# choutilin/makani

Hardware: AMD Instinct MI355X
Metric: SFNO fwd+bwd samples/sec, 73ch 721x1440 (higher is better)
Workload: dtype bf16; 1 GPU; sfno_linear_73chq_sc3_layers8_edim384 fwd+bwd+Adam, 73ch 721x1440, per-GPU batch 1; global_batch=1, parallelism=h1, spectral_dtype=f32 (GEMMs as 6 bf16 MFMA products of exact 3-way operand splits), step_launch=eager, micro_batches=1, python_gc=disabled in the timed region, adam=after backward

## Files before the change

include/makani_amd.h:

```cpp
#ifndef MAKANI_AMD_H
#define MAKANI_AMD_H

#include <stdint.h>

#ifdef __cplusplus
extern "C" {
#endif

int mk_version(void);
const char* mk_last_error(void);


int mk_quadrature(int grid, int nlat, double* theta, double* weights);

int mk_legendre_kpad(int nlat);

int mk_legendre_table(int grid, int nlat, int lmax, int mmax, int with_quad_weights, float* out);

int mk_fft_twiddle_len(int nlon);
int mk_fft_twiddles(int nlon, float* out);

int mk_rfft(const void* x, int x_dtype, float* xf, const float* twiddles,
            int bc, int nlat, int nlon, int mmax, float scale0, float scale_m, float scale_h,
            void* stream);

int mk_irfft(const float* xf, void* x, int x_dtype, const float* twiddles,
             int bc, int nlat, int nlon, int mmax, float scale0, float scale_m, float scale_h,
             void* stream);

int mk_legendre_fwd(const float* xf, const float* tab, float* c,
                    int bc, int nlat, int lmax, int mmax_loc, int m_off, int mmax_glob, void* stream);

int mk_legendre_inv(const float* c, const float* tab, float* xf,
                    int bc, int nlat, int lmax, int mmax_loc, int m_off, int mmax_glob, void* stream);

long long mk_legendre_x3_bytes(int nlat, int lmax, int mmax, int inverse);
int mk_legendre_x3_split(const float* tab, void* out, int nlat, int lmax, int mmax, int inverse, void* stream);
int mk_legendre_fwd_x3(const float* xf, const void* tab_x3, float* c,
                       int bc, int nlat, int lmax, int mmax_loc, int m_off, int mmax_glob, void* stream);
int mk_legendre_inv_x3(const float* c, const void* tab_x3, float* xf,
                       int bc, int nlat, int lmax, int mmax_loc, int m_off, int mmax_glob, void* stream);

int mk_rfft_ex(const void* x, int x_dtype, float* xf, const float* twiddles, int bc, int nlat, int nlon,
               int mmax, float scale0, float scale_m, float scale_h, int xf_layout, void* stream);
int mk_irfft_ex(const float* xf, void* x, int x_dtype, const float* twiddles, int bc, int nlat, int nlon,
                int mmax, float scale0, float scale_m, float scale_h, int xf_layout, void* stream);
int mk_legendre_fwd_x3_ex(const float* xf, const void* tab_x3, float* c, int bc, int nlat, int lmax,
                          int mmax_loc, int m_off, int mmax_glob, int xf_layout, void* stream);
int mk_legendre_inv_x3_ex(const float* c, const void* tab_x3, float* xf, int bc, int nlat, int lmax,
                          int mmax_loc, int m_off, int mmax_glob, int xf_layout, void* stream);

int mk_rfft_pm(const void* x, int x_dtype, float* xf, const float* twiddles, int bc, int nlat, int nlon, int mmax,
               float scale0, float scale_m, float scale_h, int chans, int chans_per_peer, void* stream);
int mk_irfft_pm(const float* xf, void* x, int x_dtype, const float* twiddles, int bc, int nlat, int nlon, int mmax,
                float scale0, float scale_m, float scale_h, int chans, int chans_per_peer, void* stream);

int mk_irfft_sums(const float* xf, void* x, int x_dtype, const float* twiddles, int bc, int nlat, int nlon, int mmax,
                  float scale0, float scale_m, float scale_h, int xf_layout, int chans, int chans_per_peer, double* rowsums,
                  void* stream);
int mk_irfft_sums_ws(const float* xf, void* x, int x_dtype, const float* twiddles, int bc, int nlat, int nlon, int mmax,
                     float scale0, float scale_m, float scale_h, int xf_layout, int chans, int chans_per_peer, double* rowsums,
                     double* workspace, void* stream);
int mk_irfft_affine_add(const float* xf, void* x, int x_dtype, const float* twiddles, int bc, int nlat, int nlon,
                        int mmax, float scale0, float scale_m, float scale_h, int xf_layout, const void* z,
                        const float* affine, void* stream);

long long mk_latdft_table_len(int nlat, int lmax);
int mk_latdft_table(int nlat, int lmax, float* out);
int mk_latdft_fwd(const float* xf, const float* table, float* c, int nlat, int lmax, long long ncols, void* stream);
int mk_latdft_inv(const float* c, const float* table, float* xf, int nlat, int lmax, long long ncols, void* stream);

int mk_dhconv_fwd(const float* x, const float* w, float* y, int lloc, int mloc, int batch,
                  int cin, int cout, int l_off, int m_off, void* stream);
int mk_dhconv_dgrad(const float* gy, const float* w, float* gx, int lloc, int mloc, int batch,
                    int cin, int cout, int l_off, int m_off, void* stream);
int mk_dhconv_wgrad(const float* x, const float* gy, float* gw, int lloc, int mloc, int batch,
                    int cin, int cout, int l_off, int m_off, void* stream);

int mk_dhconv_fwd_x3(const float* x, const float* w, float* y, int lloc, int mloc, int batch,
                     int cin, int cout, int l_off, int m_off, void* stream);
int mk_dhconv_dgrad_x3(const float* gy, const float* w, float* gx, int lloc, int mloc, int batch,
                       int cin, int cout, int l_off, int m_off, void* stream);
int mk_dhconv_wgrad_x3(const float* x, const float* gy, float* gw, int lloc, int mloc, int batch,
                       int cin, int cout, int l_off, int m_off, void* stream);

int mk_spec_mix_fwd(const float* x, const float* w, float* y, int lloc, int mloc, int batch,
                    int cin, int cout, int l_off, int m_off, void* stream);
int mk_spec_mix_dgrad(const float* gy, const float* w, float* gx, int lloc, int mloc, int batch,
                      int cin, int cout, int l_off, int m_off, void* stream);
int mk_spec_mix_wgrad(const float* x, const float* gy, float* gw, int lloc, int mloc, int batch,
                      int cin, int cout, int l_off, int m_off, void* stream);

int mk_spec_cmlp_fwd(const float* x, const float* w, const float* bias, float* y, int lloc, int mloc, int batch, int cin,
                     int cout, int l_off, int m_off, int per_degree, int act, void* stream);
int mk_spec_cmlp_dgrad(const float* gy, const float* w, const float* a, float* gx, int lloc, int mloc, int batch, int cin,
                       int cout, int l_off, int m_off, int per_degree, int act, void* stream);
long long mk_spec_cmlp_wgrad_workspace(int lloc, int cin, int cout, int per_degree);
int mk_spec_cmlp_wgrad(const float* x, const float* gy, float* gw, void* workspace, int lloc, int mloc, int batch, int cin,
                       int cout, int l_off, int m_off, int per_degree, void* stream);
long long mk_spec_cmlp_bgrad_workspace(int lloc, int cout);
int mk_spec_cmlp_bgrad(const float* g, float* gb, void* workspace, int lloc, int mloc, int batch, int cout, int l_off,
                       int m_off, void* stream);

int mk_spec_bdmlp_fwd(const float* x, const float* w, float* y, int rows, int nb, int ib, int ob, int act, float lambda,
                      void* stream);
int mk_spec_bdmlp_dgrad(const float* gy, const float* w, const float* a, float* gx, int rows, int nb, int ib, int ob, int act,
                        void* stream);
long long mk_spec_bdmlp_wgrad_workspace(int rows, int nb, int ib, int ob);
int mk_spec_bdmlp_wgrad(const float* x, const float* gy, float* gw, void* workspace, int rows, int nb, int ib, int ob,
                        void* stream);
int mk_spec_bdmlp_mask(const float* gy, const float* s, float* out, long long n, void* stream);

int mk_diag_fwd(const float* x, const float* w, float* y, int batch, int cin, int cout, long long P, void* stream);
int mk_diag_dgrad(const float* gy, const float* w, float* gx, int batch, int cin, int cout, long long P, void* stream);
int mk_diag_wgrad(const float* x, const float* gy, float* gw, int batch, int cin, int cout, long long P, void* stream);

int mk_spec_pack(const float* c_std, float* c_prv, int bc, int lloc, int mloc, void* stream);
int mk_spec_unpack(const float* c_prv, float* c_std, int bc, int lloc, int mloc,
                   int l_off, int m_off, void* stream);

int mk_bias_gelu_fwd(const void* x, const float* bias, void* y, int dtype, int rows, int C, long long P,
                     void* stream);
int mk_bias_gelu_bwd(const void* x, const float* bias, const void* gy, void* gx, float* gbias, int dtype,
                     int rows, int C, long long P, void* stream);
int mk_affine_add(const void* r, const void* z, const float* affine, void* y, int dtype, int rows, long long P,
                  void* stream);
int mk_instnorm_fwd(const void* x, const float* weight, const float* bias, void* y, float* stats,
                    double* workspace, int dtype, int rows, int C, long long P, float eps, int fuse_gelu,
                    void* stream);
int mk_instnorm_bwd(const void* x, const void* gy, const float* stats, const float* weight, const float* bias,
                    void* gx, double* workspace, int dtype, int rows, int C, long long P, int fuse_gelu,
                    void* stream);

int mk_instnorm_fwd_ex(const void* x, const float* weight, const float* bias, void* y, float* stats,
                       double* workspace, int dtype, int rows, int C, long long P, long long count, float eps,
                       int fuse_gelu, int phase, void* stream);
int mk_instnorm_bwd_ex(const void* x, const void* gy, const float* stats, const float* weight, const float* bias,
                       void* gx, double* workspace, int dtype, int rows, int C, long long P, long long count,
                       int fuse_gelu, int phase, void* stream);
int mk_instnorm_bwd_wb(const void* x, const void* gy, const float* stats, const float* weight, const float* bias, void* gx,
                       double* workspace, float* gwb, int dtype, int C, long long P, int fuse_gelu, void* stream);

int mk_wmse_fwd(const void* pred, int dtype, const float* tar, const float* wrow, double* loss, long long rows,
                int H, int W, float scale, void* stream);
int mk_wmse_bwd(const void* pred, int dtype, const float* tar, const float* wrow, const float* gloss, void* gpred,
                long long rows, int H, int W, float scale, void* stream);

int mk_conv1x1_x3(const float* a, long long lda, const float* b, long long ldb, float* c, long long ldc, int M, int K, long long N,
                  int batch, long long sa, long long sb, long long sc, int mode, void* stream);
int mk_conv1x1_x3_bias_act(const float* a, long long lda, const float* b, long long ldb, float* c, long long ldc, int M, int K,
                           long long N, int batch, long long sb, long long sc, const float* bias, int act, void* stream);

int mk_conv1x1_wgrad(const void* gy, const void* x, float* gw, int batch, int cout, int cin, long long P,
                     void* stream);
int mk_conv1x1_wgrad_act(const void* gy, const void* x, float* gw, int batch, int cout, int cin, long long P, int x_act,
                         void* stream);
long long mk_pce_image_bytes(int M, int K);
int mk_pce_pack(const void* w, int w_dtype , int transpose, int M, int K, int ldw, void* img,
                void* stream);
int mk_pce_pack_layout(int M, int K, long long* out3);
int mk_pce_pack_batch(const void* desc_dev, int n, void* arena, long long total_elements, void* stream);
int mk_pce_gemm(const void* x, const void* wimg, void* y, const float* bias, const void* addend, const void* aux_in,
                void* aux_out, int gelu, int batch, int M, int K, long long P, void* stream);
int mk_pce_gemm_ex(const void* x, const void* wimg, void* y, const float* bias, const void* addend, const float* addend_affine,
                   const void* aux_in, void* aux_out, int gelu, double* rowstats, int batch, int M, int K, long long P,
                   void* stream);
long long mk_pce_mlp_image_bytes(int M, int Hd, int K1);
int mk_pce_mlp_pack(const void* a1, int a1_transposed, int lda1, const void* a2, int a2_transposed, int lda2,
                    int w_dtype , int M, int Hd, int K1, void* img, void* stream);
int mk_pce_mlp(const void* x, const void* wimg, void* y, void* mid_out, const void* mid_in, const float* b1, const float* b2,
               double* rowstats_y, double* rowsum_mid, int mode, int batch, int M, int Hd, int K1, long long P, void* stream);
int mk_pce_mlp_debug_stamps(unsigned long long* out512);
int mk_instnorm_coeffs(const double* sums, const float* weight, const float* bias, float* stats, float* affine, int rows,
                       int C, long long count, float eps, void* stream);
int mk_pce_debug_stamps(unsigned long long* out512);

int mk_adam_step(float* p, const float* g, float* m, float* v, long long n, float lr, float beta1, float beta2, float eps,
                 float weight_decay, int step, void* stream);

long long mk_mt_chunks(long long n);
int mk_mt_sumsq(int T, const uint64_t* x, const long long* n, double* partials, double* tsum, int clip_mode, float max_norm,
                float* norm_out, float* coef_out, float* steps, const int* inc_slots, int ninc, void* stream);
int mk_mt_norm_finish(int T, const double* tsum, int clip_mode, float max_norm, float* norm_out, float* coef_out,
                      float* steps, const int* inc_slots, int ninc, void* stream);
int mk_mt_step_inc(float* steps, const int* slots, int nslots, void* stream);
int mk_mt_scale(int T, const uint64_t* x, const long long* n, const float* coef, void* stream);
int mk_mt_adam(int T, const uint64_t* pgmv, const long long* n, const int* step_or_slot, const float* steps, float lr,
               const float* lr_dev, float beta1, float beta2, float eps, float weight_decay, int adamw, const float* coef,
               void* stream);
int mk_mt_lamb(int stage, int T, const uint64_t* pgmv, const long long* n, const int* step_or_slot, const float* steps,
               float lr, const float* lr_dev, float beta1, float beta2, float beta3, float eps, float weight_decay, int adamw,
               int bias_correction, int trust, const float* coef, double* part_p, double* part_u, double* tsum_p,
               double* tsum_u, void* stream);

long long mk_geo_metric_workspace(int B, int C, int H);
int mk_geo_metric_sums(const void* pred, int dtype, const float* tar, const float* clim, const float* wrow, double* workspace,
                       double* sums, int B, int C, int H, int W, void* stream);

long long mk_geo_lp_workspace(int B, int C, int H);
int mk_geo_lp_sums(const void* pred, int dtype, const float* tar, const float* wrow, double* workspace, double* sums, int p,
                   int B, int C, int H, int W, void* stream);
int mk_geo_lp_bwd(const void* pred, int dtype, const float* tar, const float* wrow, const float* g, void* gpred, int p,
                  int B, int C, int H, int W, void* stream);

int mk_input_assemble(const void* x, int x_dtype, const float* u, const float* stat, const float* mean, const float* std,
                      const int* mask_chans, int n_mask, int mask_src, void* out, int out_dtype, int B, int T, int C, int Cu,
                      int Cs, int H, int W, void* stream);
int mk_input_assemble_bwd(const void* gout, int g_dtype, const float* stat, const float* std, const int* mask_chans, int n_mask,
                          int mask_src, void* gx, int x_dtype, int B, int T, int C, int Cu, int Cs, int H, int W, void* stream);

long long mk_history_workspace(int B, int Cn, int H);
int mk_history_sums(const void* x, int x_dtype, const float* u, const float* wt, double* workspace, double* sums, int B, int T,
                    int C, int Cu, int H, int W, void* stream);

int mk_cos_zenith(const float* eph, const float* sin_lat, const float* cos_lat, const float* lon_rad, float* out, long long n,
                  int H, int W, void* stream);

long long mk_chan_layernorm_workspace(int B, int C, long long P);
int mk_chan_layernorm_fwd(const void* x, int x_dtype, const float* weight, const float* bias, void* y, int y_dtype,
                          float* stats, int B, int C, long long P, float eps, int fuse_gelu, void* stream);
int mk_chan_layernorm_bwd(const void* x, int x_dtype, const void* gy, int gy_dtype, const float* stats, const float* weight,
                          const float* bias, void* gx, float* workspace, float* gwb, int B, int C, long long P, int fuse_gelu,
                          void* stream);

long long mk_degree_power_workspace(int L, int M, int BC);
int mk_degree_power(const float* c, double* workspace, double* P, int L, int M, int BC, int l_off, int m_off, void* stream);
int mk_degree_power_bwd(const float* c, const double* gP, float* gc, int L, int M, int BC, int l_off, int m_off, void* stream);

#ifdef __cplusplus
}
#endif
#endif
```

makani_amd/_lib.py:

```python
import ctypes
import os

import torch

from . import build as _build

_LIB = None

_c_int = ctypes.c_int
_c_float = ctypes.c_float
_vp = ctypes.c_void_p

SIGNATURES = {
    "mk_version": (_c_int, []),
    "mk_last_error": (ctypes.c_char_p, []),
    "mk_quadrature": (_c_int, [_c_int, _c_int, _vp, _vp]),
    "mk_legendre_kpad": (_c_int, [_c_int]),
    "mk_legendre_table": (_c_int, [_c_int, _c_int, _c_int, _c_int, _c_int, _vp]),
    "mk_fft_twiddle_len": (_c_int, [_c_int]),
    "mk_fft_twiddles": (_c_int, [_c_int, _vp]),
    "mk_rfft": (_c_int, [_vp, _c_int, _vp, _vp, _c_int, _c_int, _c_int, _c_int, _c_float, _c_float, _c_float, _vp]),
    "mk_irfft": (_c_int, [_vp, _vp, _c_int, _vp, _c_int, _c_int, _c_int, _c_int, _c_float, _c_float, _c_float, _vp]),
    "mk_legendre_fwd": (_c_int, [_vp, _vp, _vp, _c_int, _c_int, _c_int, _c_int, _c_int, _c_int, _vp]),
    "mk_legendre_inv": (_c_int, [_vp, _vp, _vp, _c_int, _c_int, _c_int, _c_int, _c_int, _c_int, _vp]),
    "mk_legendre_x3_bytes": (ctypes.c_longlong, [_c_int, _c_int, _c_int, _c_int]),
    "mk_legendre_x3_split": (_c_int, [_vp, _vp, _c_int, _c_int, _c_int, _c_int, _vp]),
    "mk_legendre_fwd_x3": (_c_int, [_vp, _vp, _vp, _c_int, _c_int, _c_int, _c_int, _c_int, _c_int, _vp]),
    "mk_legendre_inv_x3": (_c_int, [_vp, _vp, _vp, _c_int, _c_int, _c_int, _c_int, _c_int, _c_int, _vp]),
    "mk_rfft_ex": (_c_int, [_vp, _c_int, _vp, _vp, _c_int, _c_int, _c_int, _c_int, _c_float, _c_float, _c_float, _c_int, _vp]),
    "mk_irfft_ex": (_c_int, [_vp, _vp, _c_int, _vp, _c_int, _c_int, _c_int, _c_int, _c_float, _c_float, _c_float, _c_int, _vp]),
    "mk_rfft_pm": (_c_int, [_vp, _c_int, _vp, _vp, _c_int, _c_int, _c_int, _c_int, _c_float, _c_float, _c_float, _c_int, _c_int, _vp]),
    "mk_irfft_pm": (_c_int, [_vp, _vp, _c_int, _vp, _c_int, _c_int, _c_int, _c_int, _c_float, _c_float, _c_float, _c_int, _c_int, _vp]),
    "mk_irfft_sums": (_c_int, [_vp, _vp, _c_int, _vp, _c_int, _c_int, _c_int, _c_int, _c_float, _c_float, _c_float, _c_int, _c_int,
                               _c_int, _vp, _vp]),
    "mk_irfft_sums_ws": (_c_int, [_vp, _vp, _c_int, _vp, _c_int, _c_int, _c_int, _c_int, _c_float, _c_float, _c_float, _c_int, _c_int,
                                  _c_int, _vp, _vp, _vp]),
    "mk_irfft_affine_add": (_c_int, [_vp, _vp, _c_int, _vp, _c_int, _c_int, _c_int, _c_int, _c_float, _c_float, _c_float, _c_int,
                                     _vp, _vp, _vp]),
    "mk_legendre_fwd_x3_ex": (_c_int, [_vp, _vp, _vp, _c_int, _c_int, _c_int, _c_int, _c_int, _c_int, _c_int, _vp]),
    "mk_legendre_inv_x3_ex": (_c_int, [_vp, _vp, _vp, _c_int, _c_int, _c_int, _c_int, _c_int, _c_int, _c_int, _vp]),
    "mk_latdft_table_len": (ctypes.c_longlong, [_c_int, _c_int]),
    "mk_latdft_table": (_c_int, [_c_int, _c_int, _vp]),
    "mk_latdft_fwd": (_c_int, [_vp, _vp, _vp, _c_int, _c_int, ctypes.c_longlong, _vp]),
    "mk_latdft_inv": (_c_int, [_vp, _vp, _vp, _c_int, _c_int, ctypes.c_longlong, _vp]),
    "mk_dhconv_fwd": (_c_int, [_vp, _vp, _vp] + [_c_int] * 7 + [_vp]),
    "mk_dhconv_dgrad": (_c_int, [_vp, _vp, _vp] + [_c_int] * 7 + [_vp]),
    "mk_dhconv_wgrad": (_c_int, [_vp, _vp, _vp] + [_c_int] * 7 + [_vp]),
    "mk_dhconv_fwd_x3": (_c_int, [_vp, _vp, _vp] + [_c_int] * 7 + [_vp]),
    "mk_dhconv_dgrad_x3": (_c_int, [_vp, _vp, _vp] + [_c_int] * 7 + [_vp]),
    "mk_dhconv_wgrad_x3": (_c_int, [_vp, _vp, _vp] + [_c_int] * 7 + [_vp]),
    "mk_spec_mix_fwd": (_c_int, [_vp, _vp, _vp] + [_c_int] * 7 + [_vp]),
    "mk_spec_mix_dgrad": (_c_int, [_vp, _vp, _vp] + [_c_int] * 7 + [_vp]),
    "mk_spec_mix_wgrad": (_c_int, [_vp, _vp, _vp] + [_c_int] * 7 + [_vp]),
    "mk_spec_cmlp_fwd": (_c_int, [_vp, _vp, _vp, _vp] + [_c_int] * 9 + [_vp]),
    "mk_spec_cmlp_dgrad": (_c_int, [_vp, _vp, _vp, _vp] + [_c_int] * 9 + [_vp]),
    "mk_spec_cmlp_wgrad_workspace": (ctypes.c_longlong, [_c_int] * 4),
    "mk_spec_cmlp_wgrad": (_c_int, [_vp, _vp, _vp, _vp] + [_c_int] * 8 + [_vp]),
    "mk_spec_cmlp_bgrad_workspace": (ctypes.c_longlong, [_c_int] * 2),
    "mk_spec_cmlp_bgrad": (_c_int, [_vp, _vp, _vp] + [_c_int] * 6 + [_vp]),
    "mk_spec_bdmlp_fwd": (_c_int, [_vp, _vp, _vp] + [_c_int] * 5 + [_c_float, _vp]),
    "mk_spec_bdmlp_dgrad": (_c_int, [_vp, _vp, _vp, _vp] + [_c_int] * 5 + [_vp]),
    "mk_spec_bdmlp_wgrad_workspace": (ctypes.c_longlong, [_c_int] * 4),
    "mk_spec_bdmlp_wgrad": (_c_int, [_vp, _vp, _vp, _vp] + [_c_int] * 4 + [_vp]),
    "mk_spec_bdmlp_mask": (_c_int, [_vp, _vp, _vp, ctypes.c_longlong, _vp]),
    "mk_affine_add":(_c_int, [_vp, _vp, _vp, _vp, _c_int, _c_int, ctypes.c_longlong, _vp]),
    "mk_diag_fwd": (_c_int, [_vp, _vp, _vp, _c_int, _c_int, _c_int, ctypes.c_longlong, _vp]),
    "mk_diag_dgrad": (_c_int, [_vp, _vp, _vp, _c_int, _c_int, _c_int, ctypes.c_longlong, _vp]),
    "mk_diag_wgrad": (_c_int, [_vp, _vp, _vp, _c_int, _c_int, _c_int, ctypes.c_longlong, _vp]),
    "mk_spec_pack": (_c_int, [_vp, _vp, _c_int, _c_int, _c_int, _vp]),
    "mk_spec_unpack": (_c_int, [_vp, _vp, _c_int, _c_int, _c_int, _c_int, _c_int, _vp]),
    "mk_bias_gelu_fwd": (_c_int, [_vp, _vp, _vp, _c_int, _c_int, _c_int, ctypes.c_longlong, _vp]),
    "mk_bias_gelu_bwd": (_c_int, [_vp, _vp, _vp, _vp, _vp, _c_int, _c_int, _c_int, ctypes.c_longlong, _vp]),
    "mk_instnorm_fwd": (_c_int, [_vp, _vp, _vp, _vp, _vp, _vp, _c_int, _c_int, _c_int, ctypes.c_longlong, _c_float,
                                 _c_int, _vp]),
    "mk_instnorm_fwd_ex": (_c_int, [_vp, _vp, _vp, _vp, _vp, _vp, _c_int, _c_int, _c_int, ctypes.c_longlong,
                                    ctypes.c_longlong, _c_float, _c_int, _c_int, _vp]),
    "mk_instnorm_bwd_ex": (_c_int, [_vp, _vp, _vp, _vp, _vp, _vp, _vp, _c_int, _c_int, _c_int, ctypes.c_longlong,
                                    ctypes.c_longlong, _c_int, _c_int, _vp]),
    "mk_instnorm_bwd_wb": (_c_int, [_vp, _vp, _vp, _vp, _vp, _vp, _vp, _vp, _c_int, _c_int, ctypes.c_longlong, _c_int, _vp]),
    "mk_wmse_fwd": (_c_int, [_vp, _c_int, _vp, _vp, _vp, ctypes.c_longlong, _c_int, _c_int, _c_float, _vp]),
    "mk_wmse_bwd": (_c_int, [_vp, _c_int, _vp, _vp, _vp, _vp, ctypes.c_longlong, _c_int, _c_int, _c_float, _vp]),
    "mk_conv1x1_wgrad": (_c_int, [_vp, _vp, _vp, _c_int, _c_int, _c_int, ctypes.c_longlong, _vp]),
    "mk_conv1x1_x3": (_c_int, [_vp, ctypes.c_longlong, _vp, ctypes.c_longlong, _vp, ctypes.c_longlong, _c_int, _c_int, ctypes.c_longlong,
                               _c_int, ctypes.c_longlong, ctypes.c_longlong, ctypes.c_longlong, _c_int, _vp]),
    "mk_conv1x1_x3_bias_act": (_c_int, [_vp, ctypes.c_longlong, _vp, ctypes.c_longlong, _vp, ctypes.c_longlong, _c_int, _c_int,
                                        ctypes.c_longlong, _c_int, ctypes.c_longlong, ctypes.c_longlong, _vp, _c_int, _vp]),
    "mk_conv1x1_wgrad_act": (_c_int, [_vp, _vp, _vp, _c_int, _c_int, _c_int, ctypes.c_longlong, _c_int, _vp]),
    "mk_pce_mlp_image_bytes": (ctypes.c_longlong, [_c_int, _c_int, _c_int]),
    "mk_pce_mlp_pack": (_c_int, [_vp, _c_int, _c_int, _vp, _c_int, _c_int, _c_int, _c_int, _c_int, _c_int, _vp, _vp]),
    "mk_pce_mlp": (_c_int, [_vp, _vp, _vp, _vp, _vp, _vp, _vp, _vp, _vp, _c_int, _c_int, _c_int, _c_int, _c_int,
                            ctypes.c_longlong, _vp]),
    "mk_pce_mlp_debug_stamps": (_c_int, [_vp]),
    "mk_pce_image_bytes": (ctypes.c_longlong, [_c_int, _c_int]),
    "mk_pce_pack": (_c_int, [_vp, _c_int, _c_int, _c_int, _c_int, _c_int, _vp, _vp]),
    "mk_pce_pack_layout": (_c_int, [_c_int, _c_int, _vp]),
    "mk_pce_pack_batch": (_c_int, [_vp, _c_int, _vp, ctypes.c_longlong, _vp]),
    "mk_pce_gemm": (_c_int, [_vp, _vp, _vp, _vp, _vp, _vp, _vp, _c_int, _c_int, _c_int, _c_int, ctypes.c_longlong, _vp]),
    "mk_pce_gemm_ex": (_c_int, [_vp, _vp, _vp, _vp, _vp, _vp, _vp, _vp, _c_int, _vp, _c_int, _c_int, _c_int, ctypes.c_longlong, _vp]),
    "mk_instnorm_coeffs": (_c_int, [_vp, _vp, _vp, _vp, _vp, _c_int, _c_int, ctypes.c_longlong, ctypes.c_float, _vp]),
    "mk_pce_debug_stamps": (_c_int, [_vp]),
    "mk_adam_step": (_c_int, [_vp, _vp, _vp, _vp, ctypes.c_longlong] + [_c_float] * 5 + [_c_int, _vp]),
    "mk_instnorm_bwd": (_c_int, [_vp, _vp, _vp, _vp, _vp, _vp, _vp, _c_int, _c_int, _c_int, ctypes.c_longlong,
                                 _c_int, _vp]),
    "mk_mt_chunks": (ctypes.c_longlong, [ctypes.c_longlong]),
    "mk_mt_sumsq": (_c_int, [_c_int, _vp, _vp, _vp, _vp, _c_int, _c_float, _vp, _vp, _vp, _vp, _c_int, _vp]),
    "mk_mt_norm_finish": (_c_int, [_c_int, _vp, _c_int, _c_float, _vp, _vp, _vp, _vp, _c_int, _vp]),
    "mk_mt_step_inc": (_c_int, [_vp, _vp, _c_int, _vp]),
    "mk_mt_scale": (_c_int, [_c_int, _vp, _vp, _vp, _vp]),
    "mk_mt_adam": (_c_int, [_c_int, _vp, _vp, _vp, _vp, _c_float, _vp] + [_c_float] * 4 + [_c_int, _vp, _vp]),
    "mk_mt_lamb": (_c_int, [_c_int, _c_int, _vp, _vp, _vp, _vp, _c_float, _vp] + [_c_float] * 5 + [_c_int] * 3
                   + [_vp] * 6),
    "mk_geo_metric_workspace": (ctypes.c_longlong, [_c_int, _c_int, _c_int]),
    "mk_geo_metric_sums": (_c_int, [_vp, _c_int, _vp, _vp, _vp, _vp, _vp, _c_int, _c_int, _c_int, _c_int, _vp]),
    "mk_geo_lp_workspace": (ctypes.c_longlong, [_c_int, _c_int, _c_int]),
    "mk_geo_lp_sums": (_c_int, [_vp, _c_int, _vp, _vp, _vp, _vp] + [_c_int] * 5 + [_vp]),
    "mk_geo_lp_bwd": (_c_int, [_vp, _c_int, _vp, _vp, _vp, _vp] + [_c_int] * 5 + [_vp]),
    "mk_input_assemble": (_c_int, [_vp, _c_int, _vp, _vp, _vp, _vp, _vp, _c_int, _c_int, _vp, _c_int] + [_c_int] * 7 + [_vp]),
    "mk_input_assemble_bwd": (_c_int, [_vp, _c_int, _vp, _vp, _vp, _c_int, _c_int, _vp, _c_int] + [_c_int] * 7 + [_vp]),
    "mk_history_workspace": (ctypes.c_longlong, [_c_int, _c_int, _c_int]),
    "mk_history_sums": (_c_int, [_vp, _c_int, _vp, _vp, _vp, _vp] + [_c_int] * 6 + [_vp]),
    "mk_cos_zenith": (_c_int, [_vp, _vp, _vp, _vp, _vp, ctypes.c_longlong, _c_int, _c_int, _vp]),
    "mk_chan_layernorm_workspace": (ctypes.c_longlong, [_c_int, _c_int, ctypes.c_longlong]),
    "mk_chan_layernorm_fwd": (_c_int, [_vp, _c_int, _vp, _vp, _vp, _c_int, _vp, _c_int, _c_int, ctypes.c_longlong, _c_float,
                                       _c_int, _vp]),
    "mk_chan_layernorm_bwd": (_c_int, [_vp, _c_int, _vp, _c_int, _vp, _vp, _vp, _vp, _vp, _vp, _c_int, _c_int, ctypes.c_longlong,
                                       _c_int, _vp]),
    "mk_degree_power_workspace": (ctypes.c_longlong, [_c_int, _c_int, _c_int]),
    "mk_degree_power": (_c_int, [_vp, _vp, _vp] + [_c_int] * 5 + [_vp]),
    "mk_degree_power_bwd": (_c_int, [_vp, _vp, _vp] + [_c_int] * 5 + [_vp]),
}


def lib_path():
    return _build.LIB


def load():
    global _LIB
    if _LIB is not None:
        return _LIB
    path = _build.LIB
    override = os.environ.get("MK_LIB_OVERRIDE")
    if override:
        path = override
    elif _build.stale():
        if _build.have_hipcc():
            path = _build.build(verbose=False)
        elif not os.path.exists(path):
            raise RuntimeError(f"makani_amd: {path} is missing and hipcc is not available to build it")
        else:
            raise RuntimeError(f"makani_amd: {path} is older than its sources and hipcc is not available to rebuild it")
    try:
        lib = ctypes.CDLL(path)
    except OSError as e:
        raise RuntimeError(f"makani_amd: cannot load the HIP extension {path}: {e}") from e
    for name, (res, args) in SIGNATURES.items():
        fn = getattr(lib, name)
        fn.restype = res
        fn.argtypes = args
    _LIB = lib
    return lib


def check(rc, what=""):
    if rc != 0:
        msg = load().mk_last_error().decode("utf-8", "replace")
        raise RuntimeError(f"makani_amd {what} failed (code {rc}): {msg}")
```

makani_amd/build.py:

```python
import os
import shutil
import subprocess
import sys

HERE = os.path.dirname(os.path.abspath(__file__))
CSRC = os.path.join(HERE, "csrc")
LIB = os.path.join(HERE, "libmakani_amd.so")
STAMP = LIB + ".stamp"
SOURCES = ["host.cpp", "fft.hip", "gemm.hip", "x3_legendre.hip", "x3_spectral.hip", "x3_latdft.hip", "x3_conv.hip", "layout.hip", "diag.hip", "pointwise.hip", "conv_gemm.hip", "pce.hip", "pce_mlp.hip", "adam.hip", "optim.hip", "metrics.hip", "lploss.hip", "preproc.hip", "zenith.hip", "chnorm.hip", "specnorm.hip"]
HEADERS = ["common.h", "x3_engine.h", "fft_split.h", "pce_common.h", "gelu.h", "stream_io.h", "tile_map.h", os.path.join("..", "..", "include", "makani_amd.h")]


def _hipcc():
    for cand in (shutil.which("hipcc"), "/opt/rocm/bin/hipcc"):
        if cand and os.path.exists(cand):
            return cand
    raise RuntimeError("hipcc not found; libmakani_amd.so cannot be built")


def have_hipcc():
    return any(c and os.path.exists(c) for c in (shutil.which("hipcc"), "/opt/rocm/bin/hipcc"))


def _source_digest():
    import hashlib
    h = hashlib.sha256()
    h.update(os.environ.get("MK_EXTRA_HIPCC_FLAGS", "").encode() + b"\0")
    for rel in SOURCES + HEADERS:
        with open(os.path.join(CSRC, rel), "rb") as f:
            h.update(rel.encode() + b"\0" + f.read() + b"\0")
    return h.hexdigest()


def stale():
    if not os.path.exists(LIB) or not os.path.exists(STAMP):
        return True
    with open(STAMP) as f:
        return f.read().strip() != _source_digest()


def build(force=False, verbose=True):
    if not force and not stale():
        return LIB
    hipcc = _hipcc()
    objs = []
    bdir = os.path.join(CSRC, "build")
    os.makedirs(bdir, exist_ok=True)
    procs = []
    for src in SOURCES:
        obj = os.path.join(bdir, src + ".o")
        cmd = [hipcc, "-O3", "-std=c++20", "--offload-arch=gfx950", "-fPIC", "-x", "hip",
               "-c", os.path.join(CSRC, src), "-o", obj] + os.environ.get("MK_EXTRA_HIPCC_FLAGS", "").split()
        if verbose:
            print(" ".join(cmd), flush=True)
        procs.append((src, subprocess.Popen(cmd, stdout=subprocess.PIPE, stderr=subprocess.STDOUT, text=True)))
        objs.append(obj)
    for src, pr in procs:
        out, _ = pr.communicate()
        if pr.returncode != 0:
            raise RuntimeError(f"hipcc failed on {src}:\n{out}")
    cmd = [hipcc, "-shared", "-fPIC", "--offload-arch=gfx950", "-o", LIB] + objs
    if verbose:
        print(" ".join(cmd), flush=True)
    res = subprocess.run(cmd, stdout=subprocess.PIPE, stderr=subprocess.STDOUT, text=True)
    if res.returncode != 0:
        raise RuntimeError(f"link failed:\n{res.stdout}")
    import ctypes
    try:
        ctypes.CDLL(LIB)
    except OSError as e:
        raise RuntimeError(f"{LIB} was linked but does not load: {e}") from e
    with open(STAMP, "w") as f:
        f.write(_source_digest() + "\n")
    return LIB


if __name__ == "__main__":
    print(build(force="--force" in sys.argv))
```

makani_amd/csrc/x3_engine.h:

```cpp
#pragma once
#include "common.h"
#include "tile_map.h"
#include "../../include/makani_amd.h"

#include <cstdint>
#include <cstdlib>

namespace {

typedef float f32x16 __attribute__((ext_vector_type(16)));
typedef __bf16 bf16x8 __attribute__((ext_vector_type(8)));
typedef float x3_f2 __attribute__((ext_vector_type(2)));
typedef float x3_f4 __attribute__((ext_vector_type(4)));

constexpr int XT = 256;
constexpr int XM = 128, XN = 128, XK = 32;
constexpr int XPITCH = 208;
constexpr int XROWB = 192;
constexpr int XIMG = XM * XPITCH + 128;
constexpr int X3_LDS = 2 * XIMG;

__device__ __forceinline__ int plain_off(int r) { return r * XPITCH; }
__device__ __forceinline__ int pair_off(int r) { return ((r >> 1) + ((r & 1) << 6)) * XPITCH + ((r & 1) << 7); }

struct Split3 {
    uint32_t h, m, l;
};
__device__ __forceinline__ Split3 split3(float x) {
    Split3 s;
    s.h = __float_as_uint(x) & 0xFFFF0000u;
    const float r1 = x - __uint_as_float(s.h);
    s.m = __float_as_uint(r1) & 0xFFFF0000u;
    s.l = __float_as_uint(r1 - __uint_as_float(s.m));
    return s;
}
__device__ __forceinline__ uint32_t pack_hi(uint32_t e0, uint32_t e1) { return __builtin_amdgcn_perm(e1, e0, 0x07060302u); }

__device__ __forceinline__ void split_store8(const float (&v)[8], char* dst) {
    Split3 s[8];
#pragma unroll
    for (int i = 0; i < 8; ++i) s[i] = split3(v[i]);
    uint4 h, m, l;
    h.x = pack_hi(s[0].h, s[1].h); h.y = pack_hi(s[2].h, s[3].h); h.z = pack_hi(s[4].h, s[5].h); h.w = pack_hi(s[6].h, s[7].h);
    m.x = pack_hi(s[0].m, s[1].m); m.y = pack_hi(s[2].m, s[3].m); m.z = pack_hi(s[4].m, s[5].m); m.w = pack_hi(s[6].m, s[7].m);
    l.x = pack_hi(s[0].l, s[1].l); l.y = pack_hi(s[2].l, s[3].l); l.z = pack_hi(s[4].l, s[5].l); l.w = pack_hi(s[6].l, s[7].l);
    *reinterpret_cast<uint4*>(dst) = h;
    *reinterpret_cast<uint4*>(dst + 64) = m;
    *reinterpret_cast<uint4*>(dst + 128) = l;
}

constexpr unsigned X3_OOB = 0x80000000u;
__device__ __forceinline__ __amdgpu_buffer_rsrc_t x3_rsrc(const float* base) {
    return __builtin_amdgcn_make_buffer_rsrc(const_cast<float*>(base), 0, 0x7FFFFFFF, 0x00020000);
}
__device__ __forceinline__ float4 x3_load16(__amdgpu_buffer_rsrc_t rs, unsigned off) {
    return __builtin_bit_cast(float4, __builtin_amdgcn_raw_buffer_load_b128(rs, off, 0, 0));
}
__device__ __forceinline__ float2 x3_load8(__amdgpu_buffer_rsrc_t rs, unsigned off) {
    return __builtin_bit_cast(float2, __builtin_amdgcn_raw_buffer_load_b64(rs, off, 0, 0));
}


struct TransStager {
    const float* base;
    long long ldk;
    int k_lo, k_hi, cvalid;
    typedef float2 Regs[8];
    static __device__ __forceinline__ int row_off(int r) { return pair_off(r); }
    __device__ __forceinline__ void gload(int kt, Regs& r, int tid) const {
        const int w = tid >> 6, c = (tid & 63) * 2;
        const int k0 = kt * XK + w * 8;
        const __amdgpu_buffer_rsrc_t rs = x3_rsrc(base + (long long)kt * XK * ldk);
#pragma unroll
        for (int i = 0; i < 8; ++i) {
            const int k = k0 + i;
            const bool ok = k >= k_lo && k < k_hi && c < cvalid;
            r[i] = x3_load8(rs, ok ? (unsigned)(((long long)(w * 8 + i) * ldk + c) * 4) : X3_OOB);
        }
    }
    __device__ __forceinline__ void sstore(const Regs& r, char* img, int tid) const {
        const int w = tid >> 6, t = tid & 63;
        float a[8], b[8];
#pragma unroll
        for (int i = 0; i < 8; ++i) {
            a[i] = r[i].x;
            b[i] = r[i].y;
        }
        split_store8(a, img + t * XPITCH + w * 16);
        split_store8(b, img + (t + 64) * XPITCH + 128 + w * 16);
    }
};

__device__ __forceinline__ int quad_row(int lane) { return ((lane >> 3) & 3) + 8 * (lane >> 5) + 4 * ((lane >> 2) & 1); }

struct RowsBelow {
    static __device__ __forceinline__ bool live(int row, int rows) { return row < rows; }
};
template <class ROWS = RowsBelow>
__device__ __forceinline__ void row8_sstore(const float4 (&r)[4], char* img, int tid, int rows) {
#pragma unroll
    for (int q = 0; q < 2; ++q) {
        const int t = tid + q * XT, row = (t >> 6) * 16 + quad_row(t & 63);
        const float v[8] = {r[2 * q].x, r[2 * q].y, r[2 * q].z, r[2 * q].w, r[2 * q + 1].x, r[2 * q + 1].y, r[2 * q + 1].z, r[2 * q + 1].w};
        if (ROWS::live(row, rows)) split_store8(v, img + row * XPITCH + (t & 3) * 16);
    }
}

struct RowStager {
    const float* base;
    long long ld;
    int rows, kvalid;
    typedef float4 Regs[4];
    static __device__ __forceinline__ int row_off(int r) { return plain_off(r); }
    __device__ __forceinline__ void gload(int kt, Regs& r, int tid) const {
        const __amdgpu_buffer_rsrc_t rs = x3_rsrc(base);
#pragma unroll
        for (int q = 0; q < 2; ++q) {
            const int t = tid + q * XT, row = (t >> 6) * 16 + quad_row(t & 63), k = kt * XK + (t & 3) * 8;
            const unsigned off = (unsigned)(((long long)row * ld + k) * 4);
#pragma unroll
            for (int h = 0; h < 2; ++h)
                r[2 * q + h] = x3_load16(rs, (row < rows && k + 4 * h < kvalid) ? off + 16 * h : X3_OOB);
        }
    }
    __device__ __forceinline__ void sstore(const Regs& r, char* img, int tid) const { row8_sstore(r, img, tid, rows); }
};

__device__ __forceinline__ void x3_mfma_step(const char* As, const char* Bs, const int (&a_off)[2], const int (&b_off)[2],
                                             const bool (&live)[2], f32x16 (&acc)[2][2]) {
    constexpr int PA[6] = {2, 0, 1, 1, 0, 0}, PB[6] = {0, 2, 1, 0, 1, 0};
#pragma unroll
    for (int s = 0; s < 2; ++s) {
        bf16x8 bf[2][3];
#pragma unroll
        for (int b = 0; b < 2; ++b)
#pragma unroll
            for (int p = 0; p < 3; ++p) bf[b][p] = *reinterpret_cast<const bf16x8*>(Bs + b_off[b] + p * 64 + s * 32);
#pragma unroll
        for (int a = 0; a < 2; ++a)
            if (live[a]) {
                bf16x8 af[3];
#pragma unroll
                for (int p = 0; p < 3; ++p) af[p] = *reinterpret_cast<const bf16x8*>(As + a_off[a] + p * 64 + s * 32);
#pragma unroll
                for (int t = 0; t < 6; ++t)
#pragma unroll
                    for (int b = 0; b < 2; ++b)
                        acc[a][b] = __builtin_amdgcn_mfma_f32_32x32x16_bf16(af[PA[t]], bf[b][PB[t]], acc[a][b], 0, 0, 0);
            }
    }
}

template <class AS, class BS, class EPI>
__device__ __forceinline__ void x3_tile(const AS& as, const BS& bs, int kt0, int kt1, int rvalid, int cvalid, EPI epi,
                                        char* lds, int exp = 0) {
    const int tid = threadIdx.x, lane = tid & 63;
    const int wave = __builtin_amdgcn_readfirstlane(tid >> 6);
    const int wr = wave >> 1, wc = wave & 1;
    const int fi = lane & 31, kg = lane >> 5;
    char* As = lds;
    char* Bs = lds + XIMG;

    f32x16 acc[2][2];
#pragma unroll
    for (int a = 0; a < 2; ++a)
#pragma unroll
        for (int b = 0; b < 2; ++b)
#pragma unroll
            for (int r = 0; r < 16; ++r) acc[a][b][r] = 0.f;
    asm volatile("" : "+a"(acc[0][0]), "+a"(acc[0][1]), "+a"(acc[1][0]), "+a"(acc[1][1]));

    bool live[2];
    int a_off[2], b_off[2];
#pragma unroll
    for (int a = 0; a < 2; ++a) {
        a_off[a] = AS::row_off(wr * 64 + a * 32 + fi) + kg * 16;
        b_off[a] = BS::row_off(wc * 64 + 2 * fi + a) + kg * 16;
        if constexpr (EPI::PAIRED_BANDS) live[a] = (wr * 32 < rvalid) && (wc * 64 < cvalid);
        else live[a] = (wr * 64 + a * 32 < rvalid) && (wc * 64 < cvalid);
    }

    typename AS::Regs ra;
    typename BS::Regs rb;
    if (kt0 < kt1) {
        as.gload(kt0, ra, tid);
        bs.gload(kt0, rb, tid);
        as.sstore(ra, As, tid);
        bs.sstore(rb, Bs, tid);
        __syncthreads();
        if (kt0 + 1 < kt1) as.gload(kt0 + 1, ra, tid);
#pragma unroll
        for (int j = 0; j < 1; ++j)
            if (kt0 + 1 + j < kt1) bs.gload(kt0 + 1 + j, rb, tid);
    }
    for (int ktb = kt0; ktb < kt1; ktb += 1) {
#pragma unroll
        for (int j = 0; j < 1; ++j) {
            const int kt = ktb + j;
            if (kt >= kt1) break;
            if (!(exp & 4)) x3_mfma_step(As, Bs, a_off, b_off, live, acc);
            if (kt + 1 < kt1) {
                __syncthreads();
                if (!(exp & 2)) {
                    as.sstore(ra, As, tid);
                    bs.sstore(rb, Bs, tid);
                }
                __syncthreads();
                if (!(exp & 1)) {
                    if (kt + 2 < kt1 && !(exp & 8)) as.gload(kt + 2, ra, tid);
                    if (kt + 1 + 1 < kt1 && !(exp & 16)) bs.gload(kt + 1 + 1, rb, tid);
                }
            }
        }
    }
    epi.store(acc, wr, wc, fi, kg, rvalid, cvalid);
}


struct StoreEpi {
    float* cbase;
    long long ldc;
    static constexpr bool PAIRED_BANDS = false;
    __device__ __forceinline__ void store(const f32x16 (&acc)[2][2], int wr, int wc, int fi, int kg, int rvalid, int cvalid) const {
        const int col = wc * 64 + 2 * fi;
        if (col < cvalid) {
#pragma unroll
            for (int a = 0; a < 2; ++a)
#pragma unroll
                for (int r = 0; r < 16; ++r) {
                    const int row = wr * 64 + a * 32 + (r & 3) + 8 * (r >> 2) + 4 * kg;
                    if (row < rvalid) {
                        x3_f2 v2;
                        v2[0] = acc[a][0][r];
                        v2[1] = acc[a][1][r];
                        __builtin_nontemporal_store(v2, reinterpret_cast<x3_f2*>(cbase + (long long)row * ldc + col));
                    }
                }
        }
    }
};

struct AccumulateEpi {
    float* cbase;
    long long ldc;
    static constexpr bool PAIRED_BANDS = false;
    __device__ __forceinline__ void store(const f32x16 (&acc)[2][2], int wr, int wc, int fi, int kg, int rvalid, int cvalid) const {
        const int col = wc * 64 + 2 * fi;
        if (col < cvalid) {
#pragma unroll
            for (int a = 0; a < 2; ++a)
#pragma unroll
                for (int r = 0; r < 16; ++r) {
                    const int row = wr * 64 + a * 32 + (r & 3) + 8 * (r >> 2) + 4 * kg;
                    if (row < rvalid) {
                        float2* d = reinterpret_cast<float2*>(cbase + (long long)row * ldc + col);
                        const float2 o = *d;
                        *d = make_float2(o.x + acc[a][0][r], o.y + acc[a][1][r]);
                    }
                }
        }
    }
};

struct AtomicEpi {
    float* cbase;
    long long ldc;
    static constexpr bool PAIRED_BANDS = false;
    __device__ __forceinline__ void store(const f32x16 (&acc)[2][2], int wr, int wc, int fi, int kg, int rvalid, int cvalid) const {
        const int col = wc * 64 + 2 * fi;
        if (col < cvalid) {
#pragma unroll
            for (int a = 0; a < 2; ++a)
#pragma unroll
                for (int r = 0; r < 16; ++r) {
                    const int row = wr * 64 + a * 32 + (r & 3) + 8 * (r >> 2) + 4 * kg;
                    if (row < rvalid) {
                        atomicAdd(cbase + (long long)row * ldc + col, acc[a][0][r]);
                        if (col + 1 < cvalid) atomicAdd(cbase + (long long)row * ldc + col + 1, acc[a][1][r]);
                    }
                }
        }
    }
};

using mk::decode_block;
using mk::TileId;
[[maybe_unused]] inline long long grid_blocks(int nbatch, int tiles_m, int tiles_n) {
    return (long long)mk::ceil_div(nbatch, 8) * 8 * tiles_m * tiles_n;
}

[[maybe_unused]] inline int x3_exp() {
    static const int v = [] { const char* e = getenv("MK_X3_EXP"); return e ? atoi(e) : 0; }();
    return v;
}

template <class P>
int x3_launch(const char* who, void (*kernel)(P), long long nblk, void* stream, const P& p) {
    MK_REQUIRE_AS(who, nblk < 2147483647LL, "grid too large");
    hipLaunchKernelGGL(kernel, dim3((unsigned)nblk), dim3(XT), X3_LDS, (hipStream_t)stream, p);
    MK_LAUNCH_CHECK_AS(who);
    return 0;
}

}
```

makani_amd/csrc/x3_legendre.hip:

```cpp
#include "x3_engine.h"

namespace {

struct F32TileStager {
    const char* base;
    typedef float4 Regs[4];
    static constexpr int TILE_BYTES = XM * XK * 4;
    struct AllRows {
        static __device__ __forceinline__ bool live(int, int) { return true; }
    };
    static __device__ __forceinline__ int row_off(int r) { return plain_off(r); }
    __device__ __forceinline__ void gload(int kt, Regs& r, int tid) const {
        const float* p = reinterpret_cast<const float*>(base + (long long)kt * TILE_BYTES);
#pragma unroll
        for (int q = 0; q < 2; ++q) {
            const int t = tid + q * XT, row = (t >> 6) * 16 + quad_row(t & 63);
            const float* pr = p + row * XK + (t & 3) * 8;
            r[2 * q] = *reinterpret_cast<const float4*>(pr);
            r[2 * q + 1] = *reinterpret_cast<const float4*>(pr + 4);
        }
    }
    __device__ __forceinline__ void sstore(const Regs& r, char* img, int tid) const { row8_sstore<AllRows>(r, img, tid, XM); }
};

struct LegX3Params {
    const float* src;
    const char* tab;
    float* dst;
    int K, L, Mloc, m_off, N2;
    int RT;
    int KC;
    int tiles_n;
    int kmajor;
    int exp;
};

__global__ __launch_bounds__(XT, 3) void legendre_fwd_x3_kernel(LegX3Params p) {
    extern __shared__ __attribute__((aligned(16))) char lds_x3[];
    const TileId t = decode_block(p.Mloc, p.RT, p.tiles_n);
    if (!t.valid) return;
    const int m = t.batch, mg = p.m_off + m;
    const int l0 = mg + t.tm * XM;
    if (l0 >= p.L) return;
    const int n0 = t.tn * XN;
    F32TileStager as;
    as.base = p.tab + ((long long)mg * p.RT + t.tm) * p.KC * F32TileStager::TILE_BYTES;
    TransStager bs;
    bs.base = p.src + (p.kmajor ? (long long)m * p.N2 : (long long)m * p.K * p.N2) + n0;
    bs.ldk = p.kmajor ? (long long)p.Mloc * p.N2 : (long long)p.N2;
    bs.k_lo = 0;
    bs.k_hi = p.K;
    bs.cvalid = p.N2 - n0;
    const StoreEpi epi{p.dst + ((long long)l0 * p.Mloc + m) * p.N2 + n0, (long long)p.Mloc * p.N2};
    x3_tile(as, bs, 0, p.KC, p.L - l0, p.N2 - n0, epi, lds_x3, p.exp);
}

__global__ __launch_bounds__(XT, 3) void legendre_inv_x3_kernel(LegX3Params p) {
    extern __shared__ __attribute__((aligned(16))) char lds_x3[];
    const TileId t = decode_block(p.Mloc, p.RT, p.tiles_n);
    if (!t.valid) return;
    const int m = t.batch, mg = p.m_off + m;
    const int k0 = t.tm * XM;
    if (k0 >= p.K) return;
    const int n0 = t.tn * XN;
    F32TileStager as;
    as.base = p.tab + ((long long)mg * p.RT + t.tm) * p.KC * F32TileStager::TILE_BYTES;
    TransStager bs;
    bs.base = p.src + (long long)m * p.N2 + n0;
    bs.ldk = (long long)p.Mloc * p.N2;
    bs.k_lo = mg;
    bs.k_hi = p.L;
    bs.cvalid = p.N2 - n0;
    const int kt0 = mg >> 5;
    const StoreEpi epi{p.kmajor ? p.dst + ((long long)k0 * p.Mloc + m) * p.N2 + n0 : p.dst + ((long long)m * p.K + k0) * p.N2 + n0,
                       p.kmajor ? (long long)p.Mloc * p.N2 : (long long)p.N2};
    x3_tile(as, bs, kt0 < p.KC ? kt0 : p.KC, p.KC, p.K - k0, p.N2 - n0, epi, lds_x3, p.exp);
}

__global__ void legendre_x3_split_kernel(const float* __restrict__ tab, void* __restrict__ out, int K, int KP, int L,
                                         int M, int RT, int KC, int inverse, long long total) {
    const long long idx = (long long)blockIdx.x * blockDim.x + threadIdx.x;
    if (idx >= total) return;
    const int kk = (int)(idx & 31);
    const int r = (int)((idx >> 5) & 127);
    long long blk = idx >> 12;
    const int kc = (int)(blk % KC);
    blk /= KC;
    const int rt = (int)(blk % RT);
    const int m = (int)(blk / RT);
    int l, k;
    if (!inverse) {
        l = m + rt * XM + r;
        k = kc * XK + kk;
    } else {
        k = rt * XM + r;
        l = kc * XK + kk;
    }
    float v = 0.f;
    if (l < L && k < K) v = tab[((long long)m * L + l) * KP + k];
    reinterpret_cast<float*>(out)[idx] = v;
}

void x3_layout(int nlat, int lmax, int inverse, int* RT, int* KC) {
    if (!inverse) {
        *RT = mk::ceil_div(lmax, XM);
        *KC = mk::ceil_div(nlat, XK);
    } else {
        *RT = mk::ceil_div(nlat, XM);
        *KC = mk::ceil_div(lmax, XK);
    }
}

int legendre_x3_launch(const char* who, bool fwd, const float* src, const void* tab, float* dst, int bc, int nlat, int lmax,
                       int mmax_loc, int m_off, int mmax_glob, int xf_layout, void* stream) {
    MK_REQUIRE_AS(who, src && tab && dst, "null pointer");
    MK_REQUIRE_AS(who, bc > 0 && nlat > 0 && lmax > 0 && mmax_loc > 0, "bad sizes");
    MK_REQUIRE_AS(who, m_off >= 0 && m_off + mmax_loc <= mmax_glob, "mode shard out of range");
    MK_REQUIRE_AS(who, xf_layout == 0 || xf_layout == 1, "xf_layout must be 0 ([M][K][BC]) or 1 ([K][M][BC])");
    LegX3Params p;
    p.kmajor = xf_layout;
    p.src = src;
    p.tab = (const char*)tab;
    p.dst = dst;
    p.K = nlat;
    p.L = lmax;
    p.Mloc = mmax_loc;
    p.m_off = m_off;
    p.N2 = 2 * bc;
    x3_layout(nlat, lmax, fwd ? 0 : 1, &p.RT, &p.KC);
    p.tiles_n = mk::ceil_div(p.N2, XN);
    p.exp = x3_exp();
    const long long nblk = grid_blocks(mmax_loc, p.RT, p.tiles_n);
    MK_REQUIRE_AS(who, nblk < 2147483647LL && 33LL * p.Mloc * p.N2 * 4 < (1LL << 31),
               "operand too large: grid over 2^31 blocks, or 33 * mmax_loc * 2 * bc * 4 bytes (one k-step of the data operand) over 2^31");
    return x3_launch(who, fwd ? legendre_fwd_x3_kernel : legendre_inv_x3_kernel, nblk, stream, p);
}

}

extern "C" long long mk_legendre_x3_bytes(int nlat, int lmax, int mmax, int inverse) {
    if (nlat <= 0 || lmax <= 0 || mmax <= 0) return 0;
    int RT, KC;
    x3_layout(nlat, lmax, inverse, &RT, &KC);
    return (long long)mmax * RT * KC * F32TileStager::TILE_BYTES;
}

extern "C" int mk_legendre_x3_split(const float* tab, void* out, int nlat, int lmax, int mmax, int inverse, void* stream) {
    MK_REQUIRE(tab && out, "null pointer");
    MK_REQUIRE(nlat > 0 && lmax > 0 && mmax > 0, "bad sizes");
    int RT, KC;
    x3_layout(nlat, lmax, inverse, &RT, &KC);
    const long long total = (long long)mmax * RT * KC * XM * XK;
    const long long nblk = (total + 255) / 256;
    MK_REQUIRE(nblk < 2147483647LL, "grid too large");
    hipLaunchKernelGGL(legendre_x3_split_kernel, dim3((unsigned)nblk), dim3(256), 0, (hipStream_t)stream, tab,
                       out, nlat, mk_legendre_kpad(nlat), lmax, mmax, RT, KC, inverse, total);
    MK_LAUNCH_CHECK();
    return 0;
}

extern "C" int mk_legendre_fwd_x3_ex(const float* xf, const void* tab_x3, float* c, int bc, int nlat, int lmax,
                                     int mmax_loc, int m_off, int mmax_glob, int xf_layout, void* stream) {
    return legendre_x3_launch(__func__, true, xf, tab_x3, c, bc, nlat, lmax, mmax_loc, m_off, mmax_glob, xf_layout, stream);
}

extern "C" int mk_legendre_fwd_x3(const float* xf, const void* tab_x3, float* c, int bc, int nlat, int lmax, int mmax_loc,
                                  int m_off, int mmax_glob, void* stream) {
    return mk_legendre_fwd_x3_ex(xf, tab_x3, c, bc, nlat, lmax, mmax_loc, m_off, mmax_glob, 0, stream);
}

extern "C" int mk_legendre_inv_x3_ex(const float* c, const void* tab_x3, float* xf, int bc, int nlat, int lmax,
                                     int mmax_loc, int m_off, int mmax_glob, int xf_layout, void* stream) {
    return legendre_x3_launch(__func__, false, c, tab_x3, xf, bc, nlat, lmax, mmax_loc, m_off, mmax_glob, xf_layout, stream);
}

extern "C" int mk_legendre_inv_x3(const float* c, const void* tab_x3, float* xf, int bc, int nlat, int lmax, int mmax_loc,
                                  int m_off, int mmax_glob, void* stream) {
    return mk_legendre_inv_x3_ex(c, tab_x3, xf, bc, nlat, lmax, mmax_loc, m_off, mmax_glob, 0, stream);
}
```

makani_amd/csrc/x3_spectral.hip:

```cpp
#include "x3_engine.h"

namespace {

__device__ __forceinline__ int tri_rows(int Mloc, int B, int l_off, int m_off, int l) {
    int nm = l_off + l - m_off + 1;
    nm = nm < 0 ? 0 : (nm > Mloc ? Mloc : nm);
    return nm * B;
}

struct DegreeWalk {
    long long lpitch;
    int l0, KPL;
    int Mloc, B, l_off, m_off;
    __device__ __forceinline__ const float* step(const float* base, int kt, int w, int& kk0, int& rows) const {
        const int li = kt / KPL, l = l0 + li;
        kk0 = (kt - li * KPL) * (XK / 2) + w * 4;
        rows = tri_rows(Mloc, B, l_off, m_off, l);
        return base + (long long)l * lpitch;
    }
};

template <bool CONJ_B, bool WALK = false>
struct CplxStager {
    const float* base;
    long long ldk;
    int kk_hi = 0, ovalid;
    DegreeWalk walk = {};
    typedef float2 Regs[4];
    static __device__ __forceinline__ int row_off(int r) { return pair_off(r); }
    __device__ __forceinline__ void gload(int kt, Regs& r, int tid) const {
        const int w = __builtin_amdgcn_readfirstlane(tid >> 6), o = tid & 63;
        int kk0, hi;
        const float* b = base;
        if constexpr (WALK) {
            b = walk.step(base, kt, w, kk0, hi);
        } else {
            kk0 = kt * (XK / 2) + w * 4;
            hi = kk_hi;
        }
        const bool ook = o < ovalid;
        const __amdgpu_buffer_rsrc_t rs = x3_rsrc(b);
#pragma unroll
        for (int i = 0; i < 4; ++i)
            r[i] = x3_load8(rs, (ook && kk0 + i < hi) ? (unsigned)((((long long)(kk0 + i)) * ldk + o) * 8) : X3_OOB);
    }
    __device__ __forceinline__ void sstore(const Regs& r, char* img, int tid) const {
        const int w = tid >> 6, t = tid & 63;
        float a[8], b[8];
#pragma unroll
        for (int i = 0; i < 4; ++i) {
            const float re = r[i].x, im = r[i].y;
            a[2 * i] = re;
            a[2 * i + 1] = CONJ_B ? im : -im;
            b[2 * i] = im;
            b[2 * i + 1] = CONJ_B ? -re : re;
        }
        split_store8(a, img + t * XPITCH + w * 16);
        split_store8(b, img + (t + 64) * XPITCH + 128 + w * 16);
    }
};

struct DgradStager {
    const float* base;
    int O, ivalid;
    typedef float4 Regs[2];
    static __device__ __forceinline__ int row_off(int r) { return pair_off(r); }
    __device__ __forceinline__ void gload(int kt, Regs& r, int tid) const {
        const int i = (tid >> 6) * 16 + quad_row(tid & 63), o = kt * (XK / 2) + (tid & 3) * 4;
        const __amdgpu_buffer_rsrc_t rs = x3_rsrc(base);
        const unsigned off = (unsigned)(((long long)i * O + o) * 8);
#pragma unroll
        for (int h = 0; h < 2; ++h) r[h] = x3_load16(rs, (i < ivalid && o + 2 * h < O) ? off + 16 * h : X3_OOB);
    }
    __device__ __forceinline__ void sstore(const Regs& r, char* img, int tid) const {
        const int i = (tid >> 6) * 16 + quad_row(tid & 63), c = tid & 3;
        const float a[8] = {r[0].x, r[0].y, r[0].z, r[0].w, r[1].x, r[1].y, r[1].z, r[1].w};
        const float b[8] = {-r[0].y, r[0].x, -r[0].w, r[0].z, -r[1].y, r[1].x, -r[1].w, r[1].z};
        split_store8(a, img + i * XPITCH + c * 16);
        split_store8(b, img + (i + 64) * XPITCH + 128 + c * 16);
    }
};

template <bool PAIR, bool WALK>
struct ChanKStager {
    const float* base;
    long long C;
    int r_hi = 0, cvalid;
    DegreeWalk walk = {};
    typedef float2 Regs[8];
    static __device__ __forceinline__ int row_off(int r) { return PAIR ? pair_off(r) : plain_off(r); }
    __device__ __forceinline__ void gload(int kt, Regs& r, int tid) const {
        const int w = __builtin_amdgcn_readfirstlane(tid >> 6), t = tid & 63;
        int r0, hi;
        const float* b = base;
        if constexpr (WALK) {
            b = walk.step(base, kt, w, r0, hi);
        } else {
            r0 = kt * (XK / 2) + w * 4;
            hi = r_hi;
        }
        const __amdgpu_buffer_rsrc_t rs = x3_rsrc(b);
#pragma unroll
        for (int e = 0; e < 2; ++e) {
            const int c = t + 64 * e;
            const bool cok = c < cvalid;
#pragma unroll
            for (int j = 0; j < 4; ++j)
                r[4 * e + j] = x3_load8(rs, (cok && r0 + j < hi) ? (unsigned)((((long long)(r0 + j)) * C + c) * 8) : X3_OOB);
        }
    }
    __device__ __forceinline__ void sstore(const Regs& r, char* img, int tid) const {
        const int w = tid >> 6, t = tid & 63;
#pragma unroll
        for (int e = 0; e < 2; ++e) {
            const float v[8] = {r[4 * e].x, r[4 * e].y, r[4 * e + 1].x, r[4 * e + 1].y,
                                r[4 * e + 2].x, r[4 * e + 2].y, r[4 * e + 3].x, r[4 * e + 3].y};
            split_store8(v, img + row_off(t + 64 * e) + w * 16);
        }
    }
};

struct PanelParams {
    const float* a;
    const float* b;
    float* dst;
    const float* bias;
    const float* aux;
    long long ws;
    int Lloc, Mloc, B, I, O, l_off, m_off, tiles_m, tiles_n;
    int act;
    int exp;
    int G, ngroups;
};


struct CplxBiasReluEpi {
    float* cbase;
    long long ldc;
    const float* bias;
    int act;
    static constexpr bool PAIRED_BANDS = false;
    __device__ __forceinline__ CplxBiasReluEpi(const PanelParams& p, long long off, long long ldc_, int n0)
        : cbase(p.dst + off), ldc(ldc_), bias(p.bias ? p.bias + n0 : nullptr), act(p.act) {}
    __device__ __forceinline__ void store(const f32x16 (&acc)[2][2], int wr, int wc, int fi, int kg, int rvalid, int cvalid) const {
        const int col = wc * 64 + 2 * fi;
        if (col < cvalid) {
            const bool relu_re = act >= 1, relu_im = act == 2;
            float b0 = 0.f, b1 = 0.f;
            if (bias) {
                b0 = bias[col];
                b1 = bias[col + 1];
            }
#pragma unroll
            for (int a = 0; a < 2; ++a)
#pragma unroll
                for (int r = 0; r < 16; ++r) {
                    const int row = wr * 64 + a * 32 + (r & 3) + 8 * (r >> 2) + 4 * kg;
                    if (row < rvalid) {
                        x3_f2 v2;
                        v2[0] = acc[a][0][r] + b0;
                        v2[1] = acc[a][1][r] + b1;
                        if (relu_re) v2[0] = v2[0] > 0.f ? v2[0] : 0.f;
                        if (relu_im) v2[1] = v2[1] > 0.f ? v2[1] : 0.f;
                        *reinterpret_cast<x3_f2*>(cbase + (long long)row * ldc + col) = v2;
                    }
                }
        }
    }
};

struct CplxMaskEpi {
    float* cbase;
    long long ldc;
    const float* aux;
    int act;
    static constexpr bool PAIRED_BANDS = false;
    __device__ __forceinline__ CplxMaskEpi(const PanelParams& p, long long off, long long ldc_, int)
        : cbase(p.dst + off), ldc(ldc_), aux(p.aux + off), act(p.act) {}
    __device__ __forceinline__ void store(const f32x16 (&acc)[2][2], int wr, int wc, int fi, int kg, int rvalid, int cvalid) const {
        const int col = wc * 64 + 2 * fi;
        const bool both = act == 2;
        if (col < cvalid) {
#pragma unroll
            for (int a = 0; a < 2; ++a)
#pragma unroll
                for (int r = 0; r < 16; ++r) {
                    const int row = wr * 64 + a * 32 + (r & 3) + 8 * (r >> 2) + 4 * kg;
                    if (row < rvalid) {
                        const long long off = (long long)row * ldc + col;
                        x3_f2 v2;
                        const float2 m = *reinterpret_cast<const float2*>(aux + off);
                        v2[0] = m.x > 0.f ? acc[a][0][r] : 0.f;
                        v2[1] = (!both || m.y > 0.f) ? acc[a][1][r] : 0.f;
                        *reinterpret_cast<x3_f2*>(cbase + off) = v2;
                    }
                }
        }
    }
};

struct PanelStoreEpi : StoreEpi {
    __device__ __forceinline__ PanelStoreEpi(const PanelParams& p, long long off, long long ldc_, int) : StoreEpi{p.dst + off, ldc_} {}
};


template <class EPI, bool ABLATE>
__global__ __launch_bounds__(XT, 3) void dhconv_fwd_x3_kernel(PanelParams p) {
    extern __shared__ __attribute__((aligned(16))) char lds_x3[];
    const TileId t = decode_block(p.Lloc, p.tiles_m, p.tiles_n);
    if (!t.valid) return;
    const int l = p.Lloc - 1 - t.batch;
    const int R = tri_rows(p.Mloc, p.B, p.l_off, p.m_off, l);
    const int r0 = t.tm * XM;
    if (r0 >= R) return;
    const int n0 = t.tn * XN;
    const long long rowbase = (long long)l * p.Mloc * p.B + r0;
    RowStager as;
    as.base = p.a + rowbase * 2 * p.I;
    as.ld = 2 * p.I;
    as.rows = R - r0;
    as.kvalid = 2 * p.I;
    CplxStager<false> bs;
    bs.base = p.b + ((long long)l * p.ws + n0 / 2) * 2;
    bs.ldk = p.O;
    bs.kk_hi = p.I;
    bs.ovalid = p.O - n0 / 2;
    const EPI epi(p, rowbase * 2 * p.O + n0, 2LL * p.O, n0);
    x3_tile(as, bs, 0, (2 * p.I + XK - 1) / XK, R - r0, 2 * p.O - n0, epi, lds_x3, ABLATE ? p.exp : 0);
}

template <class EPI, bool ABLATE>
__global__ __launch_bounds__(XT, 3) void dhconv_dgrad_x3_kernel(PanelParams p) {
    extern __shared__ __attribute__((aligned(16))) char lds_x3[];
    const TileId t = decode_block(p.Lloc, p.tiles_m, p.tiles_n);
    if (!t.valid) return;
    const int l = p.Lloc - 1 - t.batch;
    const int R = tri_rows(p.Mloc, p.B, p.l_off, p.m_off, l);
    const int r0 = t.tm * XM;
    if (r0 >= R) return;
    const int n0 = t.tn * XN;
    const long long rowbase = (long long)l * p.Mloc * p.B + r0;
    RowStager as;
    as.base = p.a + rowbase * 2 * p.O;
    as.ld = 2 * p.O;
    as.rows = R - r0;
    as.kvalid = 2 * p.O;
    DgradStager bs;
    bs.base = p.b + ((long long)l * p.ws + (long long)(n0 / 2) * p.O) * 2;
    bs.O = p.O;
    bs.ivalid = p.I - n0 / 2;
    const EPI epi(p, rowbase * 2 * p.I + n0, 2LL * p.I, n0);
    x3_tile(as, bs, 0, (2 * p.O + XK - 1) / XK, R - r0, 2 * p.I - n0, epi, lds_x3, ABLATE ? p.exp : 0);
}

__global__ __launch_bounds__(XT, 3) void dhconv_wgrad_x3_kernel(PanelParams p) {
    extern __shared__ __attribute__((aligned(16))) char lds_x3[];
    const TileId t = decode_block(p.Lloc, p.tiles_m, p.tiles_n);
    if (!t.valid) return;
    const int l = p.Lloc - 1 - t.batch;
    const int R = tri_rows(p.Mloc, p.B, p.l_off, p.m_off, l);
    const int i0 = t.tm * XM;
    if (i0 >= p.I) return;
    const int n0 = t.tn * XN;
    const long long rowbase = (long long)l * p.Mloc * p.B;
    ChanKStager<false, false> as;
    as.base = p.a + (rowbase * p.I + i0) * 2;
    as.C = p.I;
    as.r_hi = R;
    as.cvalid = p.I - i0;
    CplxStager<true> bs;
    bs.base = p.b + (rowbase * p.O + n0 / 2) * 2;
    bs.ldk = p.O;
    bs.kk_hi = R;
    bs.ovalid = p.O - n0 / 2;
    const StoreEpi epi{p.dst + ((long long)l * p.I + i0) * 2 * p.O + n0, 2LL * p.O};
    x3_tile(as, bs, 0, (2 * R + XK - 1) / XK, p.I - i0, 2 * p.O - n0, epi, lds_x3, p.exp);
}

__global__ __launch_bounds__(XT, 3) void spec_cmlp_wgrad_shared_kernel(PanelParams p) {
    extern __shared__ __attribute__((aligned(16))) char lds_x3[];
    const TileId t = decode_block(p.ngroups, p.tiles_m, p.tiles_n);
    if (!t.valid) return;
    const int g = p.ngroups - 1 - t.batch;
    const int l0 = g * p.G, l1 = l0 + p.G < p.Lloc ? l0 + p.G : p.Lloc;
    const int KPL = (tri_rows(p.Mloc, p.B, p.l_off, p.m_off, l1 - 1) + XK / 2 - 1) / (XK / 2);
    const int i0 = t.tm * XM, n0 = t.tn * XN;
    if (i0 >= p.I) return;
    ChanKStager<false, true> as;
    as.base = p.a + 2 * i0;
    as.C = p.I;
    as.cvalid = p.I - i0;
    as.walk = {2LL * p.Mloc * p.B * p.I, l0, KPL > 0 ? KPL : 1, p.Mloc, p.B, p.l_off, p.m_off};
    CplxStager<true, true> bs;
    bs.base = p.b + n0;
    bs.ldk = p.O;
    bs.ovalid = p.O - n0 / 2;
    bs.walk = as.walk;
    bs.walk.lpitch = 2LL * p.Mloc * p.B * p.O;
    const StoreEpi epi{p.dst + ((long long)g * p.I + i0) * 2 * p.O + n0, 2LL * p.O};
    x3_tile(as, bs, 0, (l1 - l0) * KPL, p.I - i0, 2 * p.O - n0, epi, lds_x3);
}

__global__ void spec_cmlp_group_sum_kernel(const float4* __restrict__ part, float4* __restrict__ dst, long long n4, int ngroups) {
    const long long e = (long long)blockIdx.x * blockDim.x + threadIdx.x;
    if (e >= n4) return;
    float4 s = part[e];
    int g = 1;
    for (; g + 8 <= ngroups; g += 8) {
        float4 v[8];
#pragma unroll
        for (int j = 0; j < 8; ++j) v[j] = part[(long long)(g + j) * n4 + e];
#pragma unroll
        for (int j = 0; j < 8; ++j) {
            s.x += v[j].x;
            s.y += v[j].y;
            s.z += v[j].z;
            s.w += v[j].w;
        }
    }
    for (; g < ngroups; ++g) {
        const float4 v = part[(long long)g * n4 + e];
        s.x += v.x;
        s.y += v.y;
        s.z += v.z;
        s.w += v.w;
    }
    dst[e] = s;
}

__global__ __launch_bounds__(256) void spec_cmlp_bgrad_rows_kernel(const float* __restrict__ g, double* __restrict__ part, int Mloc,
                                                                   int B, int O2, int l_off, int m_off, int chunks) {
    const int l = blockIdx.x / chunks, c = (blockIdx.x - l * chunks) * 256 + threadIdx.x;
    if (c >= O2) return;
    const int R = tri_rows(Mloc, B, l_off, m_off, l);
    const float* p = g + (long long)l * Mloc * B * O2 + c;
    double s[4] = {0.0, 0.0, 0.0, 0.0};
    int r = 0;
    for (; r + 4 <= R; r += 4)
#pragma unroll
        for (int j = 0; j < 4; ++j) s[j] += (double)p[(long long)(r + j) * O2];
    for (int j = 0; r < R; ++r, ++j) s[j] += (double)p[(long long)r * O2];
    part[(long long)l * O2 + c] = (s[0] + s[1]) + (s[2] + s[3]);
}

__global__ void spec_cmlp_bgrad_sum_kernel(const double* __restrict__ part, float* __restrict__ gb, int Lloc, int O2) {
    const int c = blockIdx.x * blockDim.x + threadIdx.x;
    if (c >= O2) return;
    double s = 0.0;
    for (int l = 0; l < Lloc; ++l) s += part[(long long)l * O2 + c];
    gb[c] = (float)s;
}

int cmlp_group_size(int lloc, int cin, int cout) {
    const long long tiles = (long long)mk::ceil_div(cin, XM) * mk::ceil_div(2 * cout, XN);
    const long long G = mk::ceil_div_ll((long long)lloc * tiles, 768LL);
    return (int)(G < 1 ? 1 : G);
}

struct MixParams {
    const float* a;
    const float* w;
    float* dst;
    int Lloc, Mloc, B, Ca, Cd;
    int l_off, m_off, tiles_m, tiles_n;
    int G, ngroups;
};

struct SpecRowStager {
    const float* base;
    long long ld;
    int rows, cvalid;
    typedef float4 Regs[4];
    static __device__ __forceinline__ int row_off(int r) { return pair_off(r); }
    __device__ __forceinline__ void gload(int kt, Regs& r, int tid) const {
        const __amdgpu_buffer_rsrc_t rs = x3_rsrc(base);
        const int row = (tid >> 6) * 16 + quad_row(tid & 63), i = kt * XK + (tid & 3) * 8;
        const unsigned off = (unsigned)(((long long)row * ld + 2 * i) * 4);
#pragma unroll
        for (int h = 0; h < 4; ++h) r[h] = x3_load16(rs, (row < rows && i + 2 * h < cvalid) ? off + 16 * h : X3_OOB);
    }
    __device__ __forceinline__ void sstore(const Regs& r, char* img, int tid) const {
        const int row = (tid >> 6) * 16 + quad_row(tid & 63), c = tid & 3;
        const float re[8] = {r[0].x, r[0].z, r[1].x, r[1].z, r[2].x, r[2].z, r[3].x, r[3].z};
        const float im[8] = {r[0].y, r[0].w, r[1].y, r[1].w, r[2].y, r[2].w, r[3].y, r[3].w};
        if (row < rows) {
            split_store8(re, img + row * XPITCH + c * 16);
            split_store8(im, img + (row + 64) * XPITCH + 128 + c * 16);
        }
    }
};

struct Row2Stager {
    const float* base;
    long long ld;
    int rows, kvalid;
    typedef float2 Regs[8];
    static __device__ __forceinline__ int row_off(int r) { return pair_off(r); }
    __device__ __forceinline__ void gload(int kt, Regs& r, int tid) const {
        const __amdgpu_buffer_rsrc_t rs = x3_rsrc(base);
#pragma unroll
        for (int q = 0; q < 2; ++q) {
            const int t = tid + q * XT, row = (t >> 6) * 16 + quad_row(t & 63), k = kt * XK + (t & 3) * 8;
            const unsigned off = (unsigned)(((long long)row * ld + k) * 4);
#pragma unroll
            for (int h = 0; h < 4; ++h)
                r[4 * q + h] = x3_load8(rs, (row < rows && k + 2 * h < kvalid) ? off + 8 * h : X3_OOB);
        }
    }
    __device__ __forceinline__ void sstore(const Regs& r, char* img, int tid) const {
#pragma unroll
        for (int q = 0; q < 2; ++q) {
            const int t = tid + q * XT, row = (t >> 6) * 16 + quad_row(t & 63);
            const float v[8] = {r[4 * q].x, r[4 * q].y, r[4 * q + 1].x, r[4 * q + 1].y,
                                r[4 * q + 2].x, r[4 * q + 2].y, r[4 * q + 3].x, r[4 * q + 3].y};
            if (row < rows) split_store8(v, img + pair_off(row) + (t & 3) * 16);
        }
    }
};

struct CplxRowsEpi {
    float* cbase;
    long long ldc;
    static constexpr bool PAIRED_BANDS = false;
    __device__ __forceinline__ void store(const f32x16 (&acc)[2][2], int wr, int wc, int fi, int kg, int rvalid, int cvalid) const {
        const int col = wc * 64 + 2 * fi;
        if (col < cvalid) {
#pragma unroll
            for (int a = 0; a < 2; ++a)
#pragma unroll
                for (int r = 0; r < 16; r += 2) {
                    const int row = wr * 64 + a * 32 + (r & 3) + 8 * (r >> 2) + 4 * kg;
                    if (row < rvalid) {
                        x3_f4 v4;
                        v4[0] = acc[a][0][r];
                        v4[1] = acc[a][0][r + 1];
                        v4[2] = acc[a][1][r];
                        v4[3] = acc[a][1][r + 1];
                        __builtin_nontemporal_store(v4, reinterpret_cast<x3_f4*>(cbase + (long long)(row >> 1) * ldc + 2 * col));
                    }
                }
        }
    }
};

template <bool TRANS>
__global__ __launch_bounds__(XT, 3) void spec_mix_x3_kernel(MixParams p) {
    extern __shared__ __attribute__((aligned(16))) char lds_x3[];
    const TileId t = decode_block(p.Lloc, p.tiles_m, p.tiles_n);
    if (!t.valid) return;
    const int l = p.Lloc - 1 - t.batch;
    const int R = tri_rows(p.Mloc, p.B, p.l_off, p.m_off, l);
    const int r0 = t.tm * (XM / 2);
    if (r0 >= R) return;
    const int n0 = t.tn * XN;
    const long long rowbase = (long long)l * p.Mloc * p.B + r0;
    SpecRowStager as;
    as.base = p.a + rowbase * 2 * p.Ca;
    as.ld = 2LL * p.Ca;
    as.rows = R - r0;
    as.cvalid = p.Ca;
    const CplxRowsEpi epi{p.dst + rowbase * 2 * p.Cd + 2 * n0, 2LL * p.Cd};
    const int kts = (p.Ca + XK - 1) / XK;
    if constexpr (TRANS) {
        TransStager bs;
        bs.base = p.w + n0;
        bs.ldk = p.Cd;
        bs.k_lo = 0;
        bs.k_hi = p.Ca;
        bs.cvalid = p.Cd - n0;
        x3_tile(as, bs, 0, kts, 2 * (R - r0), p.Cd - n0, epi, lds_x3);
    } else {
        Row2Stager bs;
        bs.base = p.w + (long long)n0 * p.Ca;
        bs.ld = p.Ca;
        bs.rows = p.Cd - n0;
        bs.kvalid = p.Ca;
        x3_tile(as, bs, 0, kts, 2 * (R - r0), p.Cd - n0, epi, lds_x3);
    }
}

__global__ __launch_bounds__(XT, 3) void spec_mix_wgrad_x3_kernel(MixParams p) {
    extern __shared__ __attribute__((aligned(16))) char lds_x3[];
    const TileId t = decode_block(p.ngroups, p.tiles_m, p.tiles_n);
    if (!t.valid) return;
    const int g = p.ngroups - 1 - t.batch;
    const int l0 = g * p.G, l1 = l0 + p.G < p.Lloc ? l0 + p.G : p.Lloc;
    const int KPL = (tri_rows(p.Mloc, p.B, p.l_off, p.m_off, l1 - 1) + XK / 2 - 1) / (XK / 2);
    if (KPL == 0) return;
    const int o0 = t.tm * XM, i0 = t.tn * XN;
    ChanKStager<false, true> as;
    as.base = p.a + 2 * o0;
    as.C = p.Ca;
    as.cvalid = p.Ca - o0;
    as.walk = {2LL * p.Mloc * p.B * p.Ca, l0, KPL, p.Mloc, p.B, p.l_off, p.m_off};
    ChanKStager<true, true> bs;
    bs.base = p.w + 2 * i0;
    bs.C = p.Cd;
    bs.cvalid = p.Cd - i0;
    bs.walk = as.walk;
    bs.walk.lpitch = 2LL * p.Mloc * p.B * p.Cd;
    const AtomicEpi epi{p.dst + (long long)o0 * p.Cd + i0, p.Cd};
    x3_tile(as, bs, 0, (l1 - l0) * KPL, p.Ca - o0, p.Cd - i0, epi, lds_x3);
}

struct BlockParams {
    const float* a;
    const float* b;
    float* dst;
    const float* aux;
    int rows, nb, ib, ob, tiles_m, tiles_n;
    float lambda;
    int rg, ngroups;
};

constexpr int BD_STORE = 0, BD_RELU = 2, BD_SHRINK = 3, BD_MASK = 4;

template <int MODE>
struct BlockEpi {
    float* cbase;
    long long ldc;
    const float* aux;
    float lambda;
    static constexpr bool PAIRED_BANDS = false;
    static __device__ __forceinline__ float shrink(float v, float l) { return v > l ? v - l : (v < -l ? v + l : 0.f); }
    __device__ __forceinline__ void store(const f32x16 (&acc)[2][2], int wr, int wc, int fi, int kg, int rvalid, int cvalid) const {
        const int col = wc * 64 + 2 * fi;
        if (col < cvalid) {
#pragma unroll
            for (int a = 0; a < 2; ++a)
#pragma unroll
                for (int r = 0; r < 16; ++r) {
                    const int row = wr * 64 + a * 32 + (r & 3) + 8 * (r >> 2) + 4 * kg;
                    if (row < rvalid) {
                        const long long off = (long long)row * ldc + col;
                        x3_f2 v2;
                        v2[0] = acc[a][0][r];
                        v2[1] = acc[a][1][r];
                        if constexpr (MODE == BD_RELU) {
                            v2[0] = v2[0] > 0.f ? v2[0] : 0.f;
                            v2[1] = v2[1] > 0.f ? v2[1] : 0.f;
                        } else if constexpr (MODE == BD_SHRINK) {
                            v2[0] = shrink(v2[0], lambda);
                            v2[1] = shrink(v2[1], lambda);
                        } else if constexpr (MODE == BD_MASK) {
                            const float2 m = *reinterpret_cast<const float2*>(aux + off);
                            v2[0] = m.x > 0.f ? v2[0] : 0.f;
                            v2[1] = m.y > 0.f ? v2[1] : 0.f;
                        }
                        *reinterpret_cast<x3_f2*>(cbase + off) = v2;
                    }
                }
        }
    }
};

template <int MODE>
__global__ __launch_bounds__(XT, 3) void spec_bdmlp_fwd_kernel(BlockParams p) {
    extern __shared__ __attribute__((aligned(16))) char lds_x3[];
    const TileId t = decode_block(p.nb, p.tiles_m, p.tiles_n);
    if (!t.valid) return;
    const int k = t.batch, r0 = t.tm * XM, n0 = t.tn * XN;
    const long long ci = (long long)p.nb * p.ib, co = (long long)p.nb * p.ob;
    RowStager as;
    as.base = p.a + ((long long)r0 * ci + (long long)k * p.ib) * 2;
    as.ld = 2 * ci;
    as.rows = p.rows - r0;
    as.kvalid = 2 * p.ib;
    CplxStager<false> bs;
    bs.base = p.b + ((long long)k * p.ib * p.ob + n0 / 2) * 2;
    bs.ldk = p.ob;
    bs.kk_hi = p.ib;
    bs.ovalid = p.ob - n0 / 2;
    const BlockEpi<MODE> epi{p.dst + ((long long)r0 * co + (long long)k * p.ob) * 2 + n0, 2 * co, nullptr, p.lambda};
    x3_tile(as, bs, 0, (2 * p.ib + XK - 1) / XK, p.rows - r0, 2 * p.ob - n0, epi, lds_x3);
}

template <int MODE>
__global__ __launch_bounds__(XT, 3) void spec_bdmlp_dgrad_kernel(BlockParams p) {
    extern __shared__ __attribute__((aligned(16))) char lds_x3[];
    const TileId t = decode_block(p.nb, p.tiles_m, p.tiles_n);
    if (!t.valid) return;
    const int k = t.batch, r0 = t.tm * XM, n0 = t.tn * XN;
    const long long ci = (long long)p.nb * p.ib, co = (long long)p.nb * p.ob;
    RowStager as;
    as.base = p.a + ((long long)r0 * co + (long long)k * p.ob) * 2;
    as.ld = 2 * co;
    as.rows = p.rows - r0;
    as.kvalid = 2 * p.ob;
    DgradStager bs;
    bs.base = p.b + ((long long)k * p.ib * p.ob + (long long)(n0 / 2) * p.ob) * 2;
    bs.O = p.ob;
    bs.ivalid = p.ib - n0 / 2;
    const long long off = ((long long)r0 * ci + (long long)k * p.ib) * 2 + n0;
    const BlockEpi<MODE> epi{p.dst + off, 2 * ci, MODE == BD_MASK ? p.aux + off : nullptr, 0.f};
    x3_tile(as, bs, 0, (2 * p.ob + XK - 1) / XK, p.rows - r0, 2 * p.ib - n0, epi, lds_x3);
}

__global__ __launch_bounds__(XT, 3) void spec_bdmlp_wgrad_kernel(BlockParams p) {
    extern __shared__ __attribute__((aligned(16))) char lds_x3[];
    const TileId t = decode_block(p.nb * p.ngroups, p.tiles_m, p.tiles_n);
    if (!t.valid) return;
    const int g = t.batch / p.nb, k = t.batch - g * p.nb;
    const int i0 = t.tm * XM, n0 = t.tn * XN;
    const long long ci = (long long)p.nb * p.ib, co = (long long)p.nb * p.ob;
    const long long rbeg = (long long)g * p.rg;
    const int rcnt = p.rows - rbeg < p.rg ? (int)(p.rows - rbeg) : p.rg;
    ChanKStager<false, false> as;
    as.base = p.a + (rbeg * ci + (long long)k * p.ib + i0) * 2;
    as.C = ci;
    as.r_hi = rcnt;
    as.cvalid = p.ib - i0;
    CplxStager<true> bs;
    bs.base = p.b + (rbeg * co + (long long)k * p.ob + n0 / 2) * 2;
    bs.ldk = co;
    bs.kk_hi = rcnt;
    bs.ovalid = p.ob - n0 / 2;
    const StoreEpi epi{p.dst + (((long long)g * p.nb + k) * p.ib + i0) * 2 * p.ob + n0, 2LL * p.ob};
    x3_tile(as, bs, 0, (2 * rcnt + XK - 1) / XK, p.ib - i0, 2 * p.ob - n0, epi, lds_x3);
}

__global__ void spec_bdmlp_mask_kernel(const float4* __restrict__ gy, const float4* __restrict__ s, float4* __restrict__ out,
                                       long long n4) {
    const long long e = (long long)blockIdx.x * blockDim.x + threadIdx.x;
    if (e >= n4) return;
    const float4 g = gy[e], m = s[e];
    out[e] = make_float4(m.x != 0.f ? g.x : 0.f, m.y != 0.f ? g.y : 0.f, m.z != 0.f ? g.z : 0.f, m.w != 0.f ? g.w : 0.f);
}

int bdmlp_group_rows(int rows, int nb, int ib, int ob) {
    const long long tiles = (long long)nb * mk::ceil_div(ib, XM) * mk::ceil_div(2 * ob, XN);
    const long long want = tiles >= 512 ? 1 : 512 / tiles;
    return (int)(mk::ceil_div_ll(mk::ceil_div_ll(rows, want), 16) * 16);
}

}

static int dh_x3_check(const void* a, const void* b, const void* c, int lloc, int mloc, int batch, int cin, int cout,
                       int l_off, int m_off) {
    MK_REQUIRE(a && b && c, "null pointer");
    MK_REQUIRE(lloc > 0 && mloc > 0 && batch > 0 && cin > 0 && cout > 0, "bad sizes");
    MK_REQUIRE(l_off >= 0 && m_off >= 0, "negative shard offset");
    MK_REQUIRE(cin % 2 == 0 && cout % 2 == 0, "the bf16x3 dhconv kernels need even channel counts (use the fp32 kernels)");
    return 0;
}

static PanelParams panel_params(const float* a, const float* b, float* dst, int lloc, int mloc, int batch, int cin, int cout,
                                int l_off, int m_off, int rows_m, int cols, bool per_degree = true) {
    return PanelParams{a, b, dst, nullptr, nullptr, per_degree ? (long long)cin * cout : 0LL, lloc, mloc, batch, cin, cout,
                       l_off, m_off, mk::ceil_div(rows_m, XM), mk::ceil_div(2 * cols, XN), 0, x3_exp(), 1, 0};
}

extern "C" int mk_dhconv_fwd_x3(const float* x, const float* w, float* y, int lloc, int mloc, int batch, int cin,
                                int cout, int l_off, int m_off, void* stream) {
    if (int e = dh_x3_check(x, w, y, lloc, mloc, batch, cin, cout, l_off, m_off)) return e;
    const PanelParams p = panel_params(x, w, y, lloc, mloc, batch, cin, cout, l_off, m_off, mloc * batch, cout);
    return x3_launch(__func__, dhconv_fwd_x3_kernel<PanelStoreEpi, true>, grid_blocks(lloc, p.tiles_m, p.tiles_n), stream, p);
}

extern "C" int mk_dhconv_dgrad_x3(const float* gy, const float* w, float* gx, int lloc, int mloc, int batch, int cin,
                                  int cout, int l_off, int m_off, void* stream) {
    if (int e = dh_x3_check(gy, w, gx, lloc, mloc, batch, cin, cout, l_off, m_off)) return e;
    const PanelParams p = panel_params(gy, w, gx, lloc, mloc, batch, cin, cout, l_off, m_off, mloc * batch, cin);
    return x3_launch(__func__, dhconv_dgrad_x3_kernel<PanelStoreEpi, true>, grid_blocks(lloc, p.tiles_m, p.tiles_n), stream, p);
}

extern "C" int mk_dhconv_wgrad_x3(const float* x, const float* gy, float* gw, int lloc, int mloc, int batch, int cin,
                                  int cout, int l_off, int m_off, void* stream) {
    if (int e = dh_x3_check(x, gy, gw, lloc, mloc, batch, cin, cout, l_off, m_off)) return e;
    const PanelParams p = panel_params(x, gy, gw, lloc, mloc, batch, cin, cout, l_off, m_off, cin, cout);
    return x3_launch(__func__, dhconv_wgrad_x3_kernel, grid_blocks(lloc, p.tiles_m, p.tiles_n), stream, p);
}

static int spec_mix_check(const void* a, const void* b, const void* c, int lloc, int mloc, int batch, int cin, int cout, int l_off,
                          int m_off) {
    MK_REQUIRE(a && b && c, "null pointer");
    MK_REQUIRE(lloc > 0 && mloc > 0 && batch > 0 && cin > 0 && cout > 0, "bad sizes");
    MK_REQUIRE(l_off >= 0 && m_off >= 0, "negative shard offset");
    MK_REQUIRE(cin % 2 == 0 && cout % 2 == 0, "the spectral channel mix needs even channel counts");
    MK_REQUIRE((((uintptr_t)a | (uintptr_t)b | (uintptr_t)c) & 15) == 0, "operands must be 16-byte aligned");
    const long long cmax = cin > cout ? cin : cout;
    MK_REQUIRE((long long)mloc * batch * cmax * 8 < (1LL << 31) && 33LL * cmax * 4 < (1LL << 31),
               "one degree of the spectrum must stay below 2^31 bytes");
    return 0;
}

static int spec_mix_launch(bool trans, const float* a, const float* w, float* dst, int lloc, int mloc, int batch, int ca, int cd,
                           int l_off, int m_off, void* stream) {
    const MixParams p{a, w, dst, lloc, mloc, batch, ca, cd, l_off, m_off, mk::ceil_div(mloc * batch, XM / 2), mk::ceil_div(cd, XN), 1, 0};
    return x3_launch(__func__, trans ? spec_mix_x3_kernel<true> : spec_mix_x3_kernel<false>, grid_blocks(lloc, p.tiles_m, p.tiles_n),
                     stream, p);
}

extern "C" int mk_spec_mix_fwd(const float* x, const float* w, float* y, int lloc, int mloc, int batch, int cin, int cout,
                               int l_off, int m_off, void* stream) {
    if (int e = spec_mix_check(x, w, y, lloc, mloc, batch, cin, cout, l_off, m_off)) return e;
    return spec_mix_launch(false, x, w, y, lloc, mloc, batch, cin, cout, l_off, m_off, stream);
}

extern "C" int mk_spec_mix_dgrad(const float* gy, const float* w, float* gx, int lloc, int mloc, int batch, int cin, int cout,
                                 int l_off, int m_off, void* stream) {
    if (int e = spec_mix_check(gy, w, gx, lloc, mloc, batch, cin, cout, l_off, m_off)) return e;
    return spec_mix_launch(true, gy, w, gx, lloc, mloc, batch, cout, cin, l_off, m_off, stream);
}

extern "C" int mk_spec_mix_wgrad(const float* x, const float* gy, float* gw, int lloc, int mloc, int batch, int cin, int cout,
                                 int l_off, int m_off, void* stream) {
    if (int e = spec_mix_check(x, gy, gw, lloc, mloc, batch, cin, cout, l_off, m_off)) return e;
    MixParams p{gy, x, gw, lloc, mloc, batch, cout, cin, l_off, m_off, mk::ceil_div(cout, XM), mk::ceil_div(cin, XN), 1, 0};
    long long G = (long long)lloc * p.tiles_m * p.tiles_n / 768;
    p.G = (int)(G < 1 ? 1 : (G > 8 ? 8 : G));
    p.ngroups = mk::ceil_div(lloc, p.G);
    return x3_launch(__func__, spec_mix_wgrad_x3_kernel, grid_blocks(p.ngroups, p.tiles_m, p.tiles_n), stream, p);
}

static int spec_cmlp_check(const void* a, const void* b, const void* c, int lloc, int mloc, int batch, int cin, int cout, int l_off,
                           int m_off, int per_degree, int act) {
    if (int e = spec_mix_check(a, b, c, lloc, mloc, batch, cin, cout, l_off, m_off)) return e;
    MK_REQUIRE(per_degree == 0 || per_degree == 1, "per_degree must be 0 (one shared weight panel) or 1");
    MK_REQUIRE((long long)cin * cout * 8 < (1LL << 31), "one weight panel must stay below 2^31 bytes");
    MK_REQUIRE(act >= 0 && act <= 2, "unknown activation (0 none | 1 real | 2 cartesian)");
    return 0;
}

extern "C" int mk_spec_cmlp_fwd(const float* x, const float* w, const float* bias, float* y, int lloc, int mloc, int batch, int cin,
                                int cout, int l_off, int m_off, int per_degree, int act, void* stream) {
    if (int e = spec_cmlp_check(x, w, y, lloc, mloc, batch, cin, cout, l_off, m_off, per_degree, act)) return e;
    MK_REQUIRE(((uintptr_t)bias & 7) == 0, "the bias must be 8-byte aligned");
    PanelParams p = panel_params(x, w, y, lloc, mloc, batch, cin, cout, l_off, m_off, mloc * batch, cout, per_degree);
    p.bias = bias;
    p.act = act;
    return x3_launch(__func__, dhconv_fwd_x3_kernel<CplxBiasReluEpi, false>, grid_blocks(lloc, p.tiles_m, p.tiles_n), stream, p);
}

extern "C" int mk_spec_cmlp_dgrad(const float* gy, const float* w, const float* a, float* gx, int lloc, int mloc, int batch, int cin,
                                  int cout, int l_off, int m_off, int per_degree, int act, void* stream) {
    if (int e = spec_cmlp_check(gy, w, gx, lloc, mloc, batch, cin, cout, l_off, m_off, per_degree, act)) return e;
    MK_REQUIRE(((uintptr_t)a & 15) == 0, "operands must be 16-byte aligned");
    MK_REQUIRE(a == nullptr || act != 0, "a mask operand needs an activation mode (1 real | 2 cartesian)");
    PanelParams p = panel_params(gy, w, gx, lloc, mloc, batch, cin, cout, l_off, m_off, mloc * batch, cin, per_degree);
    p.aux = a;
    p.act = act;
    return x3_launch(__func__, a ? dhconv_dgrad_x3_kernel<CplxMaskEpi, false> : dhconv_dgrad_x3_kernel<PanelStoreEpi, false>,
                     grid_blocks(lloc, p.tiles_m, p.tiles_n), stream, p);
}

extern "C" long long mk_spec_cmlp_wgrad_workspace(int lloc, int cin, int cout, int per_degree) {
    if (per_degree || lloc <= 0 || cin <= 0 || cout <= 0) return 0;
    const int ngroups = mk::ceil_div(lloc, cmlp_group_size(lloc, cin, cout));
    return ngroups > 1 ? (long long)ngroups * cin * cout * 8 : 0;
}

extern "C" int mk_spec_cmlp_wgrad(const float* x, const float* gy, float* gw, void* workspace, int lloc, int mloc, int batch, int cin,
                                  int cout, int l_off, int m_off, int per_degree, void* stream) {
    if (int e = spec_cmlp_check(x, gy, gw, lloc, mloc, batch, cin, cout, l_off, m_off, per_degree, 0)) return e;
    if (per_degree) return mk_dhconv_wgrad_x3(x, gy, gw, lloc, mloc, batch, cin, cout, l_off, m_off, stream);
    PanelParams p = panel_params(x, gy, gw, lloc, mloc, batch, cin, cout, l_off, m_off, cin, cout, false);
    p.G = cmlp_group_size(lloc, cin, cout);
    p.ngroups = mk::ceil_div(lloc, p.G);
    if (p.ngroups > 1) {
        MK_REQUIRE(workspace && ((uintptr_t)workspace & 15) == 0, "the shared weight gradient needs its 16-byte aligned workspace");
        p.dst = static_cast<float*>(workspace);
    }
    if (int e = x3_launch(__func__, spec_cmlp_wgrad_shared_kernel, grid_blocks(p.ngroups, p.tiles_m, p.tiles_n), stream, p)) return e;
    if (p.ngroups > 1) {
        const long long n4 = (long long)cin * cout / 2;
        hipLaunchKernelGGL(spec_cmlp_group_sum_kernel, dim3((unsigned)mk::ceil_div_ll(n4, 256LL)), dim3(256), 0, (hipStream_t)stream,
                           static_cast<const float4*>(workspace), reinterpret_cast<float4*>(gw), n4, p.ngroups);
        MK_LAUNCH_CHECK();
    }
    return 0;
}

extern "C" long long mk_spec_cmlp_bgrad_workspace(int lloc, int cout) {
    return lloc > 0 && cout > 0 ? (long long)lloc * cout * 2 * 8 : 0;
}

extern "C" int mk_spec_cmlp_bgrad(const float* g, float* gb, void* workspace, int lloc, int mloc, int batch, int cout, int l_off,
                                  int m_off, void* stream) {
    if (int e = spec_mix_check(g, gb, workspace, lloc, mloc, batch, cout, cout, l_off, m_off)) return e;
    const int O2 = 2 * cout, chunks = mk::ceil_div(O2, 256);
    MK_REQUIRE((long long)lloc * chunks < 2147483647LL, "grid too large");
    hipLaunchKernelGGL(spec_cmlp_bgrad_rows_kernel, dim3((unsigned)(lloc * chunks)), dim3(256), 0, (hipStream_t)stream, g,
                       static_cast<double*>(workspace), mloc, batch, O2, l_off, m_off, chunks);
    MK_LAUNCH_CHECK();
    hipLaunchKernelGGL(spec_cmlp_bgrad_sum_kernel, dim3((unsigned)mk::ceil_div(O2, 256)), dim3(256), 0, (hipStream_t)stream,
                       static_cast<const double*>(workspace), gb, lloc, O2);
    MK_LAUNCH_CHECK();
    return 0;
}

static int spec_bdmlp_check(const void* a, const void* b, const void* c, int rows, int nb, int ib, int ob) {
    MK_REQUIRE(a && b && c, "null pointer");
    MK_REQUIRE(rows > 0 && nb > 0 && ib > 0 && ob > 0, "bad sizes");
    MK_REQUIRE(ib % 2 == 0 && ob % 2 == 0, "the block MLP needs even block sizes (block offsets must stay 16-byte aligned)");
    MK_REQUIRE((((uintptr_t)a | (uintptr_t)b | (uintptr_t)c) & 15) == 0, "operands must be 16-byte aligned");
    const long long cmax = (long long)nb * (ib > ob ? ib : ob);
    MK_REQUIRE(129LL * cmax * 8 < (1LL << 31) && (long long)ib * ob * 8 < (1LL << 31),
               "one row tile of the spectrum and one weight panel must stay below 2^31 bytes");
    return 0;
}

static BlockParams bdmlp_params(const float* a, const float* b, float* dst, int rows, int nb, int ib, int ob, int rows_m, int cols) {
    return BlockParams{a, b, dst, nullptr, rows, nb, ib, ob, mk::ceil_div(rows_m, XM), mk::ceil_div(2 * cols, XN), 0.f, 0, 1};
}

extern "C" int mk_spec_bdmlp_fwd(const float* x, const float* w, float* y, int rows, int nb, int ib, int ob, int act, float lambda,
                                 void* stream) {
    if (int e = spec_bdmlp_check(x, w, y, rows, nb, ib, ob)) return e;
    MK_REQUIRE(act == 0 || act == 2 || act == 3, "unknown activation (0 none | 2 cartesian ReLU | 3 soft-shrink)");
    MK_REQUIRE(act != 3 || lambda >= 0.f, "the soft-shrink threshold must not be negative");
    BlockParams p = bdmlp_params(x, w, y, rows, nb, ib, ob, rows, ob);
    p.lambda = lambda;
    const long long nblk = grid_blocks(nb, p.tiles_m, p.tiles_n);
    if (act == 2) return x3_launch(__func__, spec_bdmlp_fwd_kernel<BD_RELU>, nblk, stream, p);
    if (act == 3) return x3_launch(__func__, spec_bdmlp_fwd_kernel<BD_SHRINK>, nblk, stream, p);
    return x3_launch(__func__, spec_bdmlp_fwd_kernel<BD_STORE>, nblk, stream, p);
}

extern "C" int mk_spec_bdmlp_dgrad(const float* gy, const float* w, const float* a, float* gx, int rows, int nb, int ib, int ob,
                                   int act, void* stream) {
    if (int e = spec_bdmlp_check(gy, w, gx, rows, nb, ib, ob)) return e;
    MK_REQUIRE(((uintptr_t)a & 15) == 0, "operands must be 16-byte aligned");
    MK_REQUIRE(act == 0 || act == 2, "unknown mask mode (0 none | 2 cartesian ReLU)");
    MK_REQUIRE((a != nullptr) == (act == 2), "the mask operand and the mask mode go together");
    BlockParams p = bdmlp_params(gy, w, gx, rows, nb, ib, ob, rows, ib);
    p.aux = a;
    return x3_launch(__func__, a ? spec_bdmlp_dgrad_kernel<BD_MASK> : spec_bdmlp_dgrad_kernel<BD_STORE>,
                     grid_blocks(nb, p.tiles_m, p.tiles_n), stream, p);
}

extern "C" long long mk_spec_bdmlp_wgrad_workspace(int rows, int nb, int ib, int ob) {
    if (rows <= 0 || nb <= 0 || ib <= 0 || ob <= 0) return 0;
    const int ngroups = mk::ceil_div(rows, bdmlp_group_rows(rows, nb, ib, ob));
    return ngroups > 1 ? (long long)ngroups * nb * ib * ob * 8 : 0;
}

extern "C" int mk_spec_bdmlp_wgrad(const float* x, const float* gy, float* gw, void* workspace, int rows, int nb, int ib, int ob,
                                   void* stream) {
    if (int e = spec_bdmlp_check(x, gy, gw, rows, nb, ib, ob)) return e;
    BlockParams p = bdmlp_params(x, gy, gw, rows, nb, ib, ob, ib, ob);
    p.rg = bdmlp_group_rows(rows, nb, ib, ob);
    p.ngroups = mk::ceil_div(rows, p.rg);
    const long long cmax = (long long)nb * (ib > ob ? ib : ob);
    MK_REQUIRE((p.rg + 16LL) * cmax * 8 < (1LL << 31), "one row group of the spectrum must stay below 2^31 bytes");
    MK_REQUIRE((long long)nb * p.ngroups < 2147483647LL, "too many row groups");
    if (p.ngroups > 1) {
        MK_REQUIRE(workspace && ((uintptr_t)workspace & 15) == 0, "the block weight gradient needs its 16-byte aligned workspace");
        p.dst = static_cast<float*>(workspace);
    }
    if (int e = x3_launch(__func__, spec_bdmlp_wgrad_kernel, grid_blocks(nb * p.ngroups, p.tiles_m, p.tiles_n), stream, p)) return e;
    if (p.ngroups > 1) {
        const long long n4 = (long long)nb * ib * ob / 2;
        hipLaunchKernelGGL(spec_cmlp_group_sum_kernel, dim3((unsigned)mk::ceil_div_ll(n4, 256LL)), dim3(256), 0, (hipStream_t)stream,
                           static_cast<const float4*>(workspace), reinterpret_cast<float4*>(gw), n4, p.ngroups);
        MK_LAUNCH_CHECK();
    }
    return 0;
}

extern "C" int mk_spec_bdmlp_mask(const float* gy, const float* s, float* out, long long n, void* stream) {
    MK_REQUIRE(gy && s && out, "null pointer");
    MK_REQUIRE(n > 0 && n % 4 == 0, "the element count must be a positive multiple of 4 floats");
    MK_REQUIRE((((uintptr_t)gy | (uintptr_t)s | (uintptr_t)out) & 15) == 0, "operands must be 16-byte aligned");
    const long long nblk = mk::ceil_div_ll(n / 4, 256LL);
    MK_REQUIRE(nblk < 2147483647LL, "grid too large");
    hipLaunchKernelGGL(spec_bdmlp_mask_kernel, dim3((unsigned)nblk), dim3(256), 0, (hipStream_t)stream,
                       reinterpret_cast<const float4*>(gy), reinterpret_cast<const float4*>(s), reinterpret_cast<float4*>(out), n / 4);
    MK_LAUNCH_CHECK();
    return 0;
}
```

Measured before the change: 24.08 samples/s.

## Add 256-row tall-tile x3 GEMM path and enable it for dhconv dgrad

Result: no change. 24.08 samples/s, median of 2 (-0.0%).

```diff
diff --git a/include/makani_amd.h b/include/makani_amd.h
--- a/include/makani_amd.h
+++ b/include/makani_amd.h
@@ -49,6 +49,11 @@
                           int mmax_loc, int m_off, int mmax_glob, int xf_layout, void* stream);
 int mk_legendre_inv_x3_ex(const float* c, const void* tab_x3, float* xf, int bc, int nlat, int lmax,
                           int mmax_loc, int m_off, int mmax_glob, int xf_layout, void* stream);
+int mk_x3_tall_route(int family);
+int mk_legendre_fwd_x3_tile(const float* xf, const void* tab_x3, float* c, int bc, int nlat, int lmax,
+                            int mmax_loc, int m_off, int mmax_glob, int xf_layout, int tall, void* stream);
+int mk_legendre_inv_x3_tile(const float* c, const void* tab_x3, float* xf, int bc, int nlat, int lmax,
+                            int mmax_loc, int m_off, int mmax_glob, int xf_layout, int tall, void* stream);
 
 int mk_rfft_pm(const void* x, int x_dtype, float* xf, const float* twiddles, int bc, int nlat, int nlon, int mmax,
                float scale0, float scale_m, float scale_h, int chans, int chans_per_peer, void* stream);
@@ -83,6 +88,10 @@
                        int cin, int cout, int l_off, int m_off, void* stream);
 int mk_dhconv_wgrad_x3(const float* x, const float* gy, float* gw, int lloc, int mloc, int batch,
                        int cin, int cout, int l_off, int m_off, void* stream);
+int mk_dhconv_fwd_x3_tile(const float* x, const float* w, float* y, int lloc, int mloc, int batch,
+                          int cin, int cout, int l_off, int m_off, int tall, void* stream);
+int mk_dhconv_dgrad_x3_tile(const float* gy, const float* w, float* gx, int lloc, int mloc, int batch,
+                            int cin, int cout, int l_off, int m_off, int tall, void* stream);
 
 int mk_spec_mix_fwd(const float* x, const float* w, float* y, int lloc, int mloc, int batch,
                     int cin, int cout, int l_off, int m_off, void* stream);
diff --git a/makani_amd/_lib.py b/makani_amd/_lib.py
--- a/makani_amd/_lib.py
+++ b/makani_amd/_lib.py
@@ -39,6 +39,9 @@
                                      _vp, _vp, _vp]),
     "mk_legendre_fwd_x3_ex": (_c_int, [_vp, _vp, _vp, _c_int, _c_int, _c_int, _c_int, _c_int, _c_int, _c_int, _vp]),
     "mk_legendre_inv_x3_ex": (_c_int, [_vp, _vp, _vp, _c_int, _c_int, _c_int, _c_int, _c_int, _c_int, _c_int, _vp]),
+    "mk_x3_tall_route": (_c_int, [_c_int]),
+    "mk_legendre_fwd_x3_tile": (_c_int, [_vp, _vp, _vp] + [_c_int] * 8 + [_vp]),
+    "mk_legendre_inv_x3_tile": (_c_int, [_vp, _vp, _vp] + [_c_int] * 8 + [_vp]),
     "mk_latdft_table_len": (ctypes.c_longlong, [_c_int, _c_int]),
     "mk_latdft_table": (_c_int, [_c_int, _c_int, _vp]),
     "mk_latdft_fwd": (_c_int, [_vp, _vp, _vp, _c_int, _c_int, ctypes.c_longlong, _vp]),
@@ -49,6 +52,8 @@
     "mk_dhconv_fwd_x3": (_c_int, [_vp, _vp, _vp] + [_c_int] * 7 + [_vp]),
     "mk_dhconv_dgrad_x3": (_c_int, [_vp, _vp, _vp] + [_c_int] * 7 + [_vp]),
     "mk_dhconv_wgrad_x3": (_c_int, [_vp, _vp, _vp] + [_c_int] * 7 + [_vp]),
+    "mk_dhconv_fwd_x3_tile": (_c_int, [_vp, _vp, _vp] + [_c_int] * 8 + [_vp]),
+    "mk_dhconv_dgrad_x3_tile": (_c_int, [_vp, _vp, _vp] + [_c_int] * 8 + [_vp]),
     "mk_spec_mix_fwd": (_c_int, [_vp, _vp, _vp] + [_c_int] * 7 + [_vp]),
     "mk_spec_mix_dgrad": (_c_int, [_vp, _vp, _vp] + [_c_int] * 7 + [_vp]),
     "mk_spec_mix_wgrad": (_c_int, [_vp, _vp, _vp] + [_c_int] * 7 + [_vp]),
diff --git a/makani_amd/build.py b/makani_amd/build.py
--- a/makani_amd/build.py
+++ b/makani_amd/build.py
@@ -7,8 +7,8 @@
 CSRC = os.path.join(HERE, "csrc")
 LIB = os.path.join(HERE, "libmakani_amd.so")
 STAMP = LIB + ".stamp"
-SOURCES = ["host.cpp", "fft.hip", "gemm.hip", "x3_legendre.hip", "x3_spectral.hip", "x3_latdft.hip", "x3_conv.hip", "layout.hip", "diag.hip", "pointwise.hip", "conv_gemm.hip", "pce.hip", "pce_mlp.hip", "adam.hip", "optim.hip", "metrics.hip", "lploss.hip", "preproc.hip", "zenith.hip", "chnorm.hip", "specnorm.hip"]
-HEADERS = ["common.h", "x3_engine.h", "fft_split.h", "pce_common.h", "gelu.h", "stream_io.h", "tile_map.h", os.path.join("..", "..", "include", "makani_amd.h")]
+SOURCES = ["host.cpp", "fft.hip", "gemm.hip", "x3_legendre.hip", "x3_legendre_tall.hip", "x3_spectral.hip", "x3_spectral_tall.hip", "x3_latdft.hip", "x3_conv.hip", "layout.hip", "diag.hip", "pointwise.hip", "conv_gemm.hip", "pce.hip", "pce_mlp.hip", "adam.hip", "optim.hip", "metrics.hip", "lploss.hip", "preproc.hip", "zenith.hip", "chnorm.hip", "specnorm.hip"]
+HEADERS = ["common.h", "x3_engine.h", "x3_legendre.h", "x3_spectral.h", "fft_split.h", "pce_common.h", "gelu.h", "stream_io.h", "tile_map.h", os.path.join("..", "..", "include", "makani_amd.h")]
 
 
 def _hipcc():
diff --git a/makani_amd/csrc/x3_engine.h b/makani_amd/csrc/x3_engine.h
--- a/makani_amd/csrc/x3_engine.h
+++ b/makani_amd/csrc/x3_engine.h
@@ -3,6 +3,7 @@
 #include "tile_map.h"
 #include "../../include/makani_amd.h"
 
+#include <atomic>
 #include <cstdint>
 #include <cstdlib>
 
@@ -216,6 +217,95 @@
     epi.store(acc, wr, wc, fi, kg, rvalid, cvalid);
 }
 
+constexpr int X3_LDS_TALL = 3 * XIMG;
+
+template <class AS, class BS, class EPI>
+__device__ __forceinline__ void x3_tile_tall(const AS& as0, const AS& as1, const BS& bs, int kt0, int kt1, int rvalid, int cvalid,
+                                             const EPI& epi0, const EPI& epi1, char* lds) {
+    static_assert(!EPI::PAIRED_BANDS, "the tall tile takes epilogues whose 32-row bands are independent");
+    const int tid = threadIdx.x, lane = tid & 63;
+    const int wave = __builtin_amdgcn_readfirstlane(tid >> 6);
+    const int wr = wave >> 1, wc = wave & 1;
+    const int fi = lane & 31, kg = lane >> 5;
+    char* A0 = lds;
+    char* A1 = lds + XIMG;
+    char* Bs = lds + 2 * XIMG;
+    const bool two = rvalid > XM;
+
+    f32x16 acc[2][2][2];
+#pragma unroll
+    for (int i = 0; i < 2; ++i)
+#pragma unroll
+        for (int a = 0; a < 2; ++a)
+#pragma unroll
+            for (int b = 0; b < 2; ++b)
+#pragma unroll
+                for (int r = 0; r < 16; ++r) acc[i][a][b][r] = 0.f;
+    asm volatile("" : "+a"(acc[0][0][0]), "+a"(acc[0][0][1]), "+a"(acc[0][1][0]), "+a"(acc[0][1][1]),
+                      "+a"(acc[1][0][0]), "+a"(acc[1][0][1]), "+a"(acc[1][1][0]), "+a"(acc[1][1][1]));
+
+    bool live0[2], live1[2];
+    int a_off[2], b_off[2];
+#pragma unroll
+    for (int a = 0; a < 2; ++a) {
+        a_off[a] = AS::row_off(wr * 64 + a * 32 + fi) + kg * 16;
+        b_off[a] = BS::row_off(wc * 64 + 2 * fi + a) + kg * 16;
+        live0[a] = (wr * 64 + a * 32 < rvalid) && (wc * 64 < cvalid);
+        live1[a] = (XM + wr * 64 + a * 32 < rvalid) && (wc * 64 < cvalid);
+    }
+
+    typename AS::Regs ra0, ra1;
+    typename BS::Regs rb;
+    if (kt0 < kt1) {
+        as0.gload(kt0, ra0, tid);
+        if (two) as1.gload(kt0, ra1, tid);
+        bs.gload(kt0, rb, tid);
+        as0.sstore(ra0, A0, tid);
+        if (two) as1.sstore(ra1, A1, tid);
+        bs.sstore(rb, Bs, tid);
+        __syncthreads();
+        if (kt0 + 1 < kt1) {
+            as0.gload(kt0 + 1, ra0, tid);
+            if (two) as1.gload(kt0 + 1, ra1, tid);
+            bs.gload(kt0 + 1, rb, tid);
+        }
+    }
+    for (int kt = kt0; kt < kt1; ++kt) {
+        x3_mfma_step(A0, Bs, a_off, b_off, live0, acc[0]);
+        if (two) x3_mfma_step(A1, Bs, a_off, b_off, live1, acc[1]);
+        if (kt + 1 < kt1) {
+            int ts = tid, tg = tid;
+            __syncthreads();
+            asm volatile("" : "+v"(ts));
+            as0.sstore(ra0, A0, ts);
+            if (two) as1.sstore(ra1, A1, ts);
+            bs.sstore(rb, Bs, ts);
+            __syncthreads();
+            if (kt + 2 < kt1) {
+                asm volatile("" : "+v"(tg));
+                as0.gload(kt + 2, ra0, tg);
+                if (two) as1.gload(kt + 2, ra1, tg);
+                bs.gload(kt + 2, rb, tg);
+            }
+        }
+    }
+    int te = tid;
+    asm volatile("" : "+v"(te));
+    const int fie = te & 31, kge = (te & 63) >> 5;
+#pragma unroll
+    for (int i = 0; i < 2; ++i) {
+        if (i == 1 && !two) break;
+        f32x16 c[2][2];
+#pragma unroll
+        for (int a = 0; a < 2; ++a)
+#pragma unroll
+            for (int b = 0; b < 2; ++b) c[a][b] = acc[i][a][b];
+        asm volatile("" : "+v"(c[0][0]), "+v"(c[0][1]), "+v"(c[1][0]), "+v"(c[1][1]) : : "memory");
+        if (i == 0) epi0.store(c, wr, wc, fie, kge, rvalid, cvalid);
+        else epi1.store(c, wr, wc, fie, kge, rvalid - XM, cvalid);
+    }
+}
+
 
 struct StoreEpi {
     float* cbase;
@@ -302,4 +392,27 @@
     return 0;
 }
 
-}
+template <auto Kernel, class P>
+int x3_launch_tall(const char* who, long long nblk, void* stream, const P& p) {
+    MK_REQUIRE_AS(who, nblk < 2147483647LL, "grid too large");
+    static std::atomic<unsigned long long> raised{0};
+    int dev = 0;
+    MK_REQUIRE_AS(who, hipGetDevice(&dev) == hipSuccess && dev >= 0 && dev < 64, "no current device");
+    if (!(raised.load(std::memory_order_acquire) & (1ULL << dev))) {
+        MK_REQUIRE_AS(who, hipFuncSetAttribute(reinterpret_cast<const void*>(Kernel), hipFuncAttributeMaxDynamicSharedMemorySize,
+                                               X3_LDS_TALL) == hipSuccess, "cannot raise the dynamic LDS limit of a tall-tile kernel");
+        raised.fetch_or(1ULL << dev, std::memory_order_release);
+    }
+    hipLaunchKernelGGL(Kernel, dim3((unsigned)nblk), dim3(XT), X3_LDS_TALL, (hipStream_t)stream, p);
+    MK_LAUNCH_CHECK_AS(who);
+    return 0;
+}
+
+constexpr bool X3_TALL_LEGENDRE_FWD = false, X3_TALL_LEGENDRE_INV = false, X3_TALL_DHCONV_FWD = false, X3_TALL_DHCONV_DGRAD = true;
+constexpr int X3_TALL_DHCONV_MODE = 1;
+[[maybe_unused]] inline bool x3_tall_auto(bool family_default) {
+    static const int v = [] { const char* e = getenv("MK_X3_TALL"); return e && *e ? (atoi(e) != 0 ? 1 : 0) : -1; }();
+    return v < 0 ? family_default : v != 0;
+}
+
+}
diff --git a/makani_amd/csrc/x3_legendre.h b/makani_amd/csrc/x3_legendre.h
--- /dev/null
+++ b/makani_amd/csrc/x3_legendre.h
@@ -0,0 +1,73 @@
+#pragma once
+#include "x3_engine.h"
+
+namespace {
+
+struct F32TileStager {
+    const char* base;
+    typedef float4 Regs[4];
+    static constexpr int TILE_BYTES = XM * XK * 4;
+    struct AllRows {
+        static __device__ __forceinline__ bool live(int, int) { return true; }
+    };
+    static __device__ __forceinline__ int row_off(int r) { return plain_off(r); }
+    __device__ __forceinline__ void gload(int kt, Regs& r, int tid) const {
+        const float* p = reinterpret_cast<const float*>(base + (long long)kt * TILE_BYTES);
+#pragma unroll
+        for (int q = 0; q < 2; ++q) {
+            const int t = tid + q * XT, row = (t >> 6) * 16 + quad_row(t & 63);
+            const float* pr = p + row * XK + (t & 3) * 8;
+            r[2 * q] = *reinterpret_cast<const float4*>(pr);
+            r[2 * q + 1] = *reinterpret_cast<const float4*>(pr + 4);
+        }
+    }
+    __device__ __forceinline__ void sstore(const Regs& r, char* img, int tid) const { row8_sstore<AllRows>(r, img, tid, XM); }
+};
+
+struct LegX3Params {
+    const float* src;
+    const char* tab;
+    float* dst;
+    int K, L, Mloc, m_off, N2;
+    int RT;
+    int KC;
+    int tiles_n;
+    int kmajor;
+    int exp;
+};
+
+[[maybe_unused]] inline void x3_layout(int nlat, int lmax, int inverse, int* RT, int* KC) {
+    if (!inverse) {
+        *RT = mk::ceil_div(lmax, XM);
+        *KC = mk::ceil_div(nlat, XK);
+    } else {
+        *RT = mk::ceil_div(nlat, XM);
+        *KC = mk::ceil_div(lmax, XK);
+    }
+}
+
+
+[[maybe_unused]] inline LegX3Params legendre_x3_params(bool fwd, const float* src, const void* tab, float* dst, int bc, int nlat,
+                                                       int lmax, int mmax_loc, int m_off, int xf_layout) {
+    LegX3Params p;
+    p.kmajor = xf_layout;
+    p.src = src;
+    p.tab = (const char*)tab;
+    p.dst = dst;
+    p.K = nlat;
+    p.L = lmax;
+    p.Mloc = mmax_loc;
+    p.m_off = m_off;
+    p.N2 = 2 * bc;
+    x3_layout(nlat, lmax, fwd ? 0 : 1, &p.RT, &p.KC);
+    p.tiles_n = mk::ceil_div(p.N2, XN);
+    p.exp = x3_exp();
+    return p;
+}
+
+}
+
+namespace mk {
+int legendre_x3_tall_launch(const char* who, bool fwd, const float* src, const void* tab, float* dst, int bc, int nlat, int lmax,
+                            int mmax_loc, int m_off, int xf_layout, void* stream);
+}
diff --git a/makani_amd/csrc/x3_legendre.hip b/makani_amd/csrc/x3_legendre.hip
--- a/makani_amd/csrc/x3_legendre.hip
+++ b/makani_amd/csrc/x3_legendre.hip
@@ -1,39 +1,6 @@
-#include "x3_engine.h"
+#include "x3_legendre.h"
 
 namespace {
-
-struct F32TileStager {
-    const char* base;
-    typedef float4 Regs[4];
-    static constexpr int TILE_BYTES = XM * XK * 4;
-    struct AllRows {
-        static __device__ __forceinline__ bool live(int, int) { return true; }
-    };
-    static __device__ __forceinline__ int row_off(int r) { return plain_off(r); }
-    __device__ __forceinline__ void gload(int kt, Regs& r, int tid) const {
-        const float* p = reinterpret_cast<const float*>(base + (long long)kt * TILE_BYTES);
-#pragma unroll
-        for (int q = 0; q < 2; ++q) {
-            const int t = tid + q * XT, row = (t >> 6) * 16 + quad_row(t & 63);
-            const float* pr = p + row * XK + (t & 3) * 8;
-            r[2 * q] = *reinterpret_cast<const float4*>(pr);
-            r[2 * q + 1] = *reinterpret_cast<const float4*>(pr + 4);
-        }
-    }
-    __device__ __forceinline__ void sstore(const Regs& r, char* img, int tid) const { row8_sstore<AllRows>(r, img, tid, XM); }
-};
-
-struct LegX3Params {
-    const float* src;
-    const char* tab;
-    float* dst;
-    int K, L, Mloc, m_off, N2;
-    int RT;
-    int KC;
-    int tiles_n;
-    int kmajor;
-    int exp;
-};
 
 __global__ __launch_bounds__(XT, 3) void legendre_fwd_x3_kernel(LegX3Params p) {
     extern __shared__ __attribute__((aligned(16))) char lds_x3[];
@@ -101,38 +68,19 @@
     reinterpret_cast<float*>(out)[idx] = v;
 }
 
-void x3_layout(int nlat, int lmax, int inverse, int* RT, int* KC) {
-    if (!inverse) {
-        *RT = mk::ceil_div(lmax, XM);
-        *KC = mk::ceil_div(nlat, XK);
-    } else {
-        *RT = mk::ceil_div(nlat, XM);
-        *KC = mk::ceil_div(lmax, XK);
-    }
-}
-
 int legendre_x3_launch(const char* who, bool fwd, const float* src, const void* tab, float* dst, int bc, int nlat, int lmax,
-                       int mmax_loc, int m_off, int mmax_glob, int xf_layout, void* stream) {
+                       int mmax_loc, int m_off, int mmax_glob, int xf_layout, int tall, void* stream) {
     MK_REQUIRE_AS(who, src && tab && dst, "null pointer");
     MK_REQUIRE_AS(who, bc > 0 && nlat > 0 && lmax > 0 && mmax_loc > 0, "bad sizes");
     MK_REQUIRE_AS(who, m_off >= 0 && m_off + mmax_loc <= mmax_glob, "mode shard out of range");
     MK_REQUIRE_AS(who, xf_layout == 0 || xf_layout == 1, "xf_layout must be 0 ([M][K][BC]) or 1 ([K][M][BC])");
-    LegX3Params p;
-    p.kmajor = xf_layout;
-    p.src = src;
-    p.tab = (const char*)tab;
-    p.dst = dst;
-    p.K = nlat;
-    p.L = lmax;
-    p.Mloc = mmax_loc;
-    p.m_off = m_off;
-    p.N2 = 2 * bc;
-    x3_layout(nlat, lmax, fwd ? 0 : 1, &p.RT, &p.KC);
-    p.tiles_n = mk::ceil_div(p.N2, XN);
-    p.exp = x3_exp();
+    MK_REQUIRE_AS(who, tall >= -1 && tall <= 1, "tall must be -1 (auto), 0 (128-row tile) or 1 (256-row tile)");
+    const LegX3Params p = legendre_x3_params(fwd, src, tab, dst, bc, nlat, lmax, mmax_loc, m_off, xf_layout);
+    if (tall < 0) tall = p.RT > 1 && x3_tall_auto(fwd ? X3_TALL_LEGENDRE_FWD : X3_TALL_LEGENDRE_INV);
     const long long nblk = grid_blocks(mmax_loc, p.RT, p.tiles_n);
     MK_REQUIRE_AS(who, nblk < 2147483647LL && 33LL * p.Mloc * p.N2 * 4 < (1LL << 31),
                "operand too large: grid over 2^31 blocks, or 33 * mmax_loc * 2 * bc * 4 bytes (one k-step of the data operand) over 2^31");
+    if (tall) return mk::legendre_x3_tall_launch(who, fwd, src, tab, dst, bc, nlat, lmax, mmax_loc, m_off, xf_layout, stream);
     return x3_launch(who, fwd ? legendre_fwd_x3_kernel : legendre_inv_x3_kernel, nblk, stream, p);
 }
 
@@ -159,9 +107,24 @@
     return 0;
 }
 
+extern "C" int mk_x3_tall_route(int family) {
+    switch (family) {
+        case 0: return x3_tall_auto(X3_TALL_LEGENDRE_FWD) ? 1 : 0;
+        case 1: return x3_tall_auto(X3_TALL_LEGENDRE_INV) ? 1 : 0;
+        case 2: return x3_tall_auto(X3_TALL_DHCONV_FWD) ? X3_TALL_DHCONV_MODE : 0;
+        case 3: return x3_tall_auto(X3_TALL_DHCONV_DGRAD) ? X3_TALL_DHCONV_MODE : 0;
+        default: return -1;
+    }
+}
+
+extern "C" int mk_legendre_fwd_x3_tile(const float* xf, const void* tab_x3, float* c, int bc, int nlat, int lmax,
+                                       int mmax_loc, int m_off, int mmax_glob, int xf_layout, int tall, void* stream) {
+    return legendre_x3_launch(__func__, true, xf, tab_x3, c, bc, nlat, lmax, mmax_loc, m_off, mmax_glob, xf_layout, tall, stream);
+}
+
 extern "C" int mk_legendre_fwd_x3_ex(const float* xf, const void* tab_x3, float* c, int bc, int nlat, int lmax,
                                      int mmax_loc, int m_off, int mmax_glob, int xf_layout, void* stream) {
-    return legendre_x3_launch(__func__, true, xf, tab_x3, c, bc, nlat, lmax, mmax_loc, m_off, mmax_glob, xf_layout, stream);
+    return legendre_x3_launch(__func__, true, xf, tab_x3, c, bc, nlat, lmax, mmax_loc, m_off, mmax_glob, xf_layout, -1, stream);
 }
 
 extern "C" int mk_legendre_fwd_x3(const float* xf, const void* tab_x3, float* c, int bc, int nlat, int lmax, int mmax_loc,
@@ -169,9 +132,14 @@
     return mk_legendre_fwd_x3_ex(xf, tab_x3, c, bc, nlat, lmax, mmax_loc, m_off, mmax_glob, 0, stream);
 }
 
+extern "C" int mk_legendre_inv_x3_tile(const float* c, const void* tab_x3, float* xf, int bc, int nlat, int lmax,
+                                       int mmax_loc, int m_off, int mmax_glob, int xf_layout, int tall, void* stream) {
+    return legendre_x3_launch(__func__, false, c, tab_x3, xf, bc, nlat, lmax, mmax_loc, m_off, mmax_glob, xf_layout, tall, stream);
+}
+
 extern "C" int mk_legendre_inv_x3_ex(const float* c, const void* tab_x3, float* xf, int bc, int nlat, int lmax,
                                      int mmax_loc, int m_off, int mmax_glob, int xf_layout, void* stream) {
-    return legendre_x3_launch(__func__, false, c, tab_x3, xf, bc, nlat, lmax, mmax_loc, m_off, mmax_glob, xf_layout, stream);
+    return legendre_x3_launch(__func__, false, c, tab_x3, xf, bc, nlat, lmax, mmax_loc, m_off, mmax_glob, xf_layout, -1, stream);
 }
 
 extern "C" int mk_legendre_inv_x3(const float* c, const void* tab_x3, float* xf, int bc, int nlat, int lmax, int mmax_loc,
diff --git a/makani_amd/csrc/x3_legendre_tall.hip b/makani_amd/csrc/x3_legendre_tall.hip
--- /dev/null
+++ b/makani_amd/csrc/x3_legendre_tall.hip
@@ -0,0 +1,60 @@
+#include "x3_legendre.h"
+
+namespace {
+
+__global__ __launch_bounds__(XT, 2) void legendre_fwd_x3_tall_kernel(LegX3Params p) {
+    extern __shared__ __attribute__((aligned(16))) char lds_x3[];
+    const TileId t = decode_block(p.Mloc, (p.RT + 1) / 2, p.tiles_n);
+    if (!t.valid) return;
+    const int m = t.batch, mg = p.m_off + m;
+    const int l0 = mg + t.tm * 2 * XM;
+    if (l0 >= p.L) return;
+    const int n0 = t.tn * XN;
+    F32TileStager as0, as1;
+    as0.base = p.tab + ((long long)mg * p.RT + 2 * t.tm) * p.KC * F32TileStager::TILE_BYTES;
+    as1.base = as0.base + (long long)p.KC * F32TileStager::TILE_BYTES;
+    TransStager bs;
+    bs.base = p.src + (p.kmajor ? (long long)m * p.N2 : (long long)m * p.K * p.N2) + n0;
+    bs.ldk = p.kmajor ? (long long)p.Mloc * p.N2 : (long long)p.N2;
+    bs.k_lo = 0;
+    bs.k_hi = p.K;
+    bs.cvalid = p.N2 - n0;
+    const long long ldc = (long long)p.Mloc * p.N2;
+    const StoreEpi epi0{p.dst + ((long long)l0 * p.Mloc + m) * p.N2 + n0, ldc};
+    const StoreEpi epi1{epi0.cbase + XM * ldc, ldc};
+    x3_tile_tall(as0, as1, bs, 0, p.KC, p.L - l0, p.N2 - n0, epi0, epi1, lds_x3);
+}
+
+__global__ __launch_bounds__(XT, 2) void legendre_inv_x3_tall_kernel(LegX3Params p) {
+    extern __shared__ __attribute__((aligned(16))) char lds_x3[];
+    const TileId t = decode_block(p.Mloc, (p.RT + 1) / 2, p.tiles_n);
+    if (!t.valid) return;
+    const int m = t.batch, mg = p.m_off + m;
+    const int k0 = t.tm * 2 * XM;
+    if (k0 >= p.K) return;
+    const int n0 = t.tn * XN;
+    F32TileStager as0, as1;
+    as0.base = p.tab + ((long long)mg * p.RT + 2 * t.tm) * p.KC * F32TileStager::TILE_BYTES;
+    as1.base = as0.base + (long long)p.KC * F32TileStager::TILE_BYTES;
+    TransStager bs;
+    bs.base = p.src + (long long)m * p.N2 + n0;
+    bs.ldk = (long long)p.Mloc * p.N2;
+    bs.k_lo = mg;
+    bs.k_hi = p.L;
+    bs.cvalid = p.N2 - n0;
+    const int kt0 = mg >> 5;
+    const long long ldc = p.kmajor ? (long long)p.Mloc * p.N2 : (long long)p.N2;
+    const StoreEpi epi0{p.kmajor ? p.dst + ((long long)k0 * p.Mloc + m) * p.N2 + n0 : p.dst + ((long long)m * p.K + k0) * p.N2 + n0, ldc};
+    const StoreEpi epi1{epi0.cbase + XM * ldc, ldc};
+    x3_tile_tall(as0, as1, bs, kt0 < p.KC ? kt0 : p.KC, p.KC, p.K - k0, p.N2 - n0, epi0, epi1, lds_x3);
+}
+
+}
+
+int mk::legendre_x3_tall_launch(const char* who, bool fwd, const float* src, const void* tab, float* dst, int bc, int nlat,
+                                int lmax, int mmax_loc, int m_off, int xf_layout, void* stream) {
+    const LegX3Params p = legendre_x3_params(fwd, src, tab, dst, bc, nlat, lmax, mmax_loc, m_off, xf_layout);
+    const long long nblk = grid_blocks(mmax_loc, (p.RT + 1) / 2, p.tiles_n);
+    return fwd ? x3_launch_tall<legendre_fwd_x3_tall_kernel>(who, nblk, stream, p)
+               : x3_launch_tall<legendre_inv_x3_tall_kernel>(who, nblk, stream, p);
+}
diff --git a/makani_amd/csrc/x3_spectral.h b/makani_amd/csrc/x3_spectral.h
--- /dev/null
+++ b/makani_amd/csrc/x3_spectral.h
@@ -0,0 +1,113 @@
+#pragma once
+#include "x3_engine.h"
+
+namespace {
+
+__device__ __forceinline__ int tri_rows(int Mloc, int B, int l_off, int m_off, int l) {
+    int nm = l_off + l - m_off + 1;
+    nm = nm < 0 ? 0 : (nm > Mloc ? Mloc : nm);
+    return nm * B;
+}
+
+struct DegreeWalk {
+    long long lpitch;
+    int l0, KPL;
+    int Mloc, B, l_off, m_off;
+    __device__ __forceinline__ const float* step(const float* base, int kt, int w, int& kk0, int& rows) const {
+        const int li = kt / KPL, l = l0 + li;
+        kk0 = (kt - li * KPL) * (XK / 2) + w * 4;
+        rows = tri_rows(Mloc, B, l_off, m_off, l);
+        return base + (long long)l * lpitch;
+    }
+};
+
+template <bool CONJ_B, bool WALK = false>
+struct CplxStager {
+    const float* base;
+    long long ldk;
+    int kk_hi = 0, ovalid;
+    DegreeWalk walk = {};
+    typedef float2 Regs[4];
+    static __device__ __forceinline__ int row_off(int r) { return pair_off(r); }
+    __device__ __forceinline__ void gload(int kt, Regs& r, int tid) const {
+        const int w = __builtin_amdgcn_readfirstlane(tid >> 6), o = tid & 63;
+        int kk0, hi;
+        const float* b = base;
+        if constexpr (WALK) {
+            b = walk.step(base, kt, w, kk0, hi);
+        } else {
+            kk0 = kt * (XK / 2) + w * 4;
+            hi = kk_hi;
+        }
+        const bool ook = o < ovalid;
+        const __amdgpu_buffer_rsrc_t rs = x3_rsrc(b);
+#pragma unroll
+        for (int i = 0; i < 4; ++i)
+            r[i] = x3_load8(rs, (ook && kk0 + i < hi) ? (unsigned)((((long long)(kk0 + i)) * ldk + o) * 8) : X3_OOB);
+    }
+    __device__ __forceinline__ void sstore(const Regs& r, char* img, int tid) const {
+        const int w = tid >> 6, t = tid & 63;
+        float a[8], b[8];
+#pragma unroll
+        for (int i = 0; i < 4; ++i) {
+            const float re = r[i].x, im = r[i].y;
+            a[2 * i] = re;
+            a[2 * i + 1] = CONJ_B ? im : -im;
+            b[2 * i] = im;
+            b[2 * i + 1] = CONJ_B ? -re : re;
+        }
+        split_store8(a, img + t * XPITCH + w * 16);
+        split_store8(b, img + (t + 64) * XPITCH + 128 + w * 16);
+    }
+};
+
+struct DgradStager {
+    const float* base;
+    int O, ivalid;
+    typedef float4 Regs[2];
+    static __device__ __forceinline__ int row_off(int r) { return pair_off(r); }
+    __device__ __forceinline__ void gload(int kt, Regs& r, int tid) const {
+        const int i = (tid >> 6) * 16 + quad_row(tid & 63), o = kt * (XK / 2) + (tid & 3) * 4;
+        const __amdgpu_buffer_rsrc_t rs = x3_rsrc(base);
+        const unsigned off = (unsigned)(((long long)i * O + o) * 8);
+#pragma unroll
+        for (int h = 0; h < 2; ++h) r[h] = x3_load16(rs, (i < ivalid && o + 2 * h < O) ? off + 16 * h : X3_OOB);
+    }
+    __device__ __forceinline__ void sstore(const Regs& r, char* img, int tid) const {
+        const int i = (tid >> 6) * 16 + quad_row(tid & 63), c = tid & 3;
+        const float a[8] = {r[0].x, r[0].y, r[0].z, r[0].w, r[1].x, r[1].y, r[1].z, r[1].w};
+        const float b[8] = {-r[0].y, r[0].x, -r[0].w, r[0].z, -r[1].y, r[1].x, -r[1].w, r[1].z};
+        split_store8(a, img + i * XPITCH + c * 16);
+        split_store8(b, img + (i + 64) * XPITCH + 128 + c * 16);
+    }
+};
+
+struct PanelParams {
+    const float* a;
+    const float* b;
+    float* dst;
+    const float* bias;
+    const float* aux;
+    long long ws;
+    int Lloc, Mloc, B, I, O, l_off, m_off, tiles_m, tiles_n;
+    int act;
+    int exp;
+    int G, ngroups;
+};
+
+struct PanelStoreEpi : StoreEpi {
+    __device__ __forceinline__ PanelStoreEpi(const PanelParams& p, long long off, long long ldc_, int) : StoreEpi{p.dst + off, ldc_} {}
+};
+
+[[maybe_unused]] inline PanelParams panel_params(const float* a, const float* b, float* dst, int lloc, int mloc, int batch, int cin, int cout,
+                                int l_off, int m_off, int rows_m, int cols, bool per_degree = true) {
+    return PanelParams{a, b, dst, nullptr, nullptr, per_degree ? (long long)cin * cout : 0LL, lloc, mloc, batch, cin, cout,
+                       l_off, m_off, mk::ceil_div(rows_m, XM), mk::ceil_div(2 * cols, XN), 0, x3_exp(), 1, 0};
+}
+
+}
+
+namespace mk {
+int dhconv_x3_tall_launch(const char* who, bool fwd, const float* a, const float* w, float* dst, int lloc, int mloc, int batch,
+                          int cin, int cout, int l_off, int m_off, int nheavy, void* stream);
+}
diff --git a/makani_amd/csrc/x3_spectral.hip b/makani_amd/csrc/x3_spectral.hip
--- a/makani_amd/csrc/x3_spectral.hip
+++ b/makani_amd/csrc/x3_spectral.hip
@@ -1,85 +1,6 @@
-#include "x3_engine.h"
+#include "x3_spectral.h"
 
 namespace {
-
-__device__ __forceinline__ int tri_rows(int Mloc, int B, int l_off, int m_off, int l) {
-    int nm = l_off + l - m_off + 1;
-    nm = nm < 0 ? 0 : (nm > Mloc ? Mloc : nm);
-    return nm * B;
-}
-
-struct DegreeWalk {
-    long long lpitch;
-    int l0, KPL;
-    int Mloc, B, l_off, m_off;
-    __device__ __forceinline__ const float* step(const float* base, int kt, int w, int& kk0, int& rows) const {
-        const int li = kt / KPL, l = l0 + li;
-        kk0 = (kt - li * KPL) * (XK / 2) + w * 4;
-        rows = tri_rows(Mloc, B, l_off, m_off, l);
-        return base + (long long)l * lpitch;
-    }
-};
-
-template <bool CONJ_B, bool WALK = false>
-struct CplxStager {
-    const float* base;
-    long long ldk;
-    int kk_hi = 0, ovalid;
-    DegreeWalk walk = {};
-    typedef float2 Regs[4];
-    static __device__ __forceinline__ int row_off(int r) { return pair_off(r); }
-    __device__ __forceinline__ void gload(int kt, Regs& r, int tid) const {
-        const int w = __builtin_amdgcn_readfirstlane(tid >> 6), o = tid & 63;
-        int kk0, hi;
-        const float* b = base;
-        if constexpr (WALK) {
-            b = walk.step(base, kt, w, kk0, hi);
-        } else {
-            kk0 = kt * (XK / 2) + w * 4;
-            hi = kk_hi;
-        }
-        const bool ook = o < ovalid;
-        const __amdgpu_buffer_rsrc_t rs = x3_rsrc(b);
-#pragma unroll
-        for (int i = 0; i < 4; ++i)
-            r[i] = x3_load8(rs, (ook && kk0 + i < hi) ? (unsigned)((((long long)(kk0 + i)) * ldk + o) * 8) : X3_OOB);
-    }
-    __device__ __forceinline__ void sstore(const Regs& r, char* img, int tid) const {
-        const int w = tid >> 6, t = tid & 63;
-        float a[8], b[8];
-#pragma unroll
-        for (int i = 0; i < 4; ++i) {
-            const float re = r[i].x, im = r[i].y;
-            a[2 * i] = re;
-            a[2 * i + 1] = CONJ_B ? im : -im;
-            b[2 * i] = im;
-            b[2 * i + 1] = CONJ_B ? -re : re;
-        }
-        split_store8(a, img + t * XPITCH + w * 16);
-        split_store8(b, img + (t + 64) * XPITCH + 128 + w * 16);
-    }
-};
-
-struct DgradStager {
-    const float* base;
-    int O, ivalid;
-    typedef float4 Regs[2];
-    static __device__ __forceinline__ int row_off(int r) { return pair_off(r); }
-    __device__ __forceinline__ void gload(int kt, Regs& r, int tid) const {
-        const int i = (tid >> 6) * 16 + quad_row(tid & 63), o = kt * (XK / 2) + (tid & 3) * 4;
-        const __amdgpu_buffer_rsrc_t rs = x3_rsrc(base);
-        const unsigned off = (unsigned)(((long long)i * O + o) * 8);
-#pragma unroll
-        for (int h = 0; h < 2; ++h) r[h] = x3_load16(rs, (i < ivalid && o + 2 * h < O) ? off + 16 * h : X3_OOB);
-    }
-    __device__ __forceinline__ void sstore(const Regs& r, char* img, int tid) const {
-        const int i = (tid >> 6) * 16 + quad_row(tid & 63), c = tid & 3;
-        const float a[8] = {r[0].x, r[0].y, r[0].z, r[0].w, r[1].x, r[1].y, r[1].z, r[1].w};
-        const float b[8] = {-r[0].y, r[0].x, -r[0].w, r[0].z, -r[1].y, r[1].x, -r[1].w, r[1].z};
-        split_store8(a, img + i * XPITCH + c * 16);
-        split_store8(b, img + (i + 64) * XPITCH + 128 + c * 16);
-    }
-};
 
 template <bool PAIR, bool WALK>
 struct ChanKStager {
@@ -120,19 +41,6 @@
     }
 };
 
-struct PanelParams {
-    const float* a;
-    const float* b;
-    float* dst;
-    const float* bias;
-    const float* aux;
-    long long ws;
-    int Lloc, Mloc, B, I, O, l_off, m_off, tiles_m, tiles_n;
-    int act;
-    int exp;
-    int G, ngroups;
-};
-
 
 struct CplxBiasReluEpi {
     float* cbase;
@@ -197,10 +105,6 @@
                 }
         }
     }
-};
-
-struct PanelStoreEpi : StoreEpi {
-    __device__ __forceinline__ PanelStoreEpi(const PanelParams& p, long long off, long long ldc_, int) : StoreEpi{p.dst + off, ldc_} {}
 };
 
 
@@ -644,24 +548,57 @@
     return 0;
 }
 
-static PanelParams panel_params(const float* a, const float* b, float* dst, int lloc, int mloc, int batch, int cin, int cout,
-                                int l_off, int m_off, int rows_m, int cols, bool per_degree = true) {
-    return PanelParams{a, b, dst, nullptr, nullptr, per_degree ? (long long)cin * cout : 0LL, lloc, mloc, batch, cin, cout,
-                       l_off, m_off, mk::ceil_div(rows_m, XM), mk::ceil_div(2 * cols, XN), 0, x3_exp(), 1, 0};
+static int dh_first_heavy(int lloc, int mloc, int batch, int l_off, int m_off) {
+    if ((long long)mloc * batch <= XM) return lloc;
+    const long long l = (long long)(XM / batch + 1) - 1 - l_off + m_off;
+    return (int)(l < 0 ? 0 : (l > lloc ? lloc : l));
+}
+
+template <bool FWD>
+static int dhconv_x3_route(const char* who, const float* a, const float* w, float* dst, int lloc, int mloc, int batch, int cin,
+                           int cout, int l_off, int m_off, int tall, void* stream) {
+    MK_REQUIRE_AS(who, tall >= -1 && tall <= 2, "tall must be -1 (auto), 0 (128-row tile), 1 (256-row tile) or 2 (by row count)");
+    const int cols = FWD ? cout : cin;
+    const int lh = dh_first_heavy(lloc, mloc, batch, l_off, m_off);
+    if (tall < 0) tall = lh < lloc && x3_tall_auto(FWD ? X3_TALL_DHCONV_FWD : X3_TALL_DHCONV_DGRAD) ? X3_TALL_DHCONV_MODE : 0;
+    if (tall == 0) {
+        const PanelParams p = panel_params(a, w, dst, lloc, mloc, batch, cin, cout, l_off, m_off, mloc * batch, cols);
+        return x3_launch(who, FWD ? dhconv_fwd_x3_kernel<PanelStoreEpi, true> : dhconv_dgrad_x3_kernel<PanelStoreEpi, true>,
+                         grid_blocks(lloc, p.tiles_m, p.tiles_n), stream, p);
+    }
+    const int nheavy = tall == 1 ? lloc : lloc - lh;
+    if (nheavy > 0)
+        if (int e = mk::dhconv_x3_tall_launch(who, FWD, a, w, dst, lloc, mloc, batch, cin, cout, l_off, m_off, nheavy, stream)) return e;
+    if (tall == 2 && lh > 0) {
+        const PanelParams p = panel_params(a, w, dst, lh, mloc, batch, cin, cout, l_off, m_off, XM, cols);
+        return x3_launch(who, FWD ? dhconv_fwd_x3_kernel<PanelStoreEpi, true> : dhconv_dgrad_x3_kernel<PanelStoreEpi, true>,
+                         grid_blocks(lh, p.tiles_m, p.tiles_n), stream, p);
+    }
+    return 0;
+}
+
+extern "C" int mk_dhconv_fwd_x3_tile(const float* x, const float* w, float* y, int lloc, int mloc, int batch, int cin,
+                                     int cout, int l_off, int m_off, int tall, void* stream) {
+    if (int e = dh_x3_check(x, w, y, lloc, mloc, batch, cin, cout, l_off, m_off)) return e;
+    return dhconv_x3_route<true>(__func__, x, w, y, lloc, mloc, batch, cin, cout, l_off, m_off, tall, stream);
+}
+
+extern "C" int mk_dhconv_dgrad_x3_tile(const float* gy, const float* w, float* gx, int lloc, int mloc, int batch, int cin,
+                                       int cout, int l_off, int m_off, int tall, void* stream) {
+    if (int e = dh_x3_check(gy, w, gx, lloc, mloc, batch, cin, cout, l_off, m_off)) return e;
+    return dhconv_x3_route<false>(__func__, gy, w, gx, lloc, mloc, batch, cin, cout, l_off, m_off, tall, stream);
 }
 
 extern "C" int mk_dhconv_fwd_x3(const float* x, const float* w, float* y, int lloc, int mloc, int batch, int cin,
                                 int cout, int l_off, int m_off, void* stream) {
     if (int e = dh_x3_check(x, w, y, lloc, mloc, batch, cin, cout, l_off, m_off)) return e;
-    const PanelParams p = panel_params(x, w, y, lloc, mloc, batch, cin, cout, l_off, m_off, mloc * batch, cout);
-    return x3_launch(__func__, dhconv_fwd_x3_kernel<PanelStoreEpi, true>, grid_blocks(lloc, p.tiles_m, p.tiles_n), stream, p);
+    return dhconv_x3_route<true>(__func__, x, w, y, lloc, mloc, batch, cin, cout, l_off, m_off, -1, stream);
 }
 
 extern "C" int mk_dhconv_dgrad_x3(const float* gy, const float* w, float* gx, int lloc, int mloc, int batch, int cin,
                                   int cout, int l_off, int m_off, void* stream) {
     if (int e = dh_x3_check(gy, w, gx, lloc, mloc, batch, cin, cout, l_off, m_off)) return e;
-    const PanelParams p = panel_params(gy, w, gx, lloc, mloc, batch, cin, cout, l_off, m_off, mloc * batch, cin);
-    return x3_launch(__func__, dhconv_dgrad_x3_kernel<PanelStoreEpi, true>, grid_blocks(lloc, p.tiles_m, p.tiles_n), stream, p);
+    return dhconv_x3_route<false>(__func__, gy, w, gx, lloc, mloc, batch, cin, cout, l_off, m_off, -1, stream);
 }
 
 extern "C" int mk_dhconv_wgrad_x3(const float* x, const float* gy, float* gw, int lloc, int mloc, int batch, int cin,
diff --git a/makani_amd/csrc/x3_spectral_tall.hip b/makani_amd/csrc/x3_spectral_tall.hip
--- /dev/null
+++ b/makani_amd/csrc/x3_spectral_tall.hip
@@ -0,0 +1,73 @@
+#include "x3_spectral.h"
+
+namespace {
+
+struct TallPanelParams : PanelParams {
+    int nheavy;
+};
+
+template <class EPI>
+__global__ __launch_bounds__(XT, 2) void dhconv_fwd_x3_tall_kernel(TallPanelParams p) {
+    extern __shared__ __attribute__((aligned(16))) char lds_x3[];
+    const TileId t = decode_block(p.nheavy, p.tiles_m, p.tiles_n);
+    if (!t.valid) return;
+    const int l = p.Lloc - 1 - t.batch;
+    const int R = tri_rows(p.Mloc, p.B, p.l_off, p.m_off, l);
+    const int r0 = t.tm * 2 * XM;
+    if (r0 >= R) return;
+    const int n0 = t.tn * XN;
+    const long long rowbase = (long long)l * p.Mloc * p.B + r0;
+    RowStager as0, as1;
+    as0.base = p.a + rowbase * 2 * p.I;
+    as0.ld = 2 * p.I;
+    as0.rows = R - r0;
+    as0.kvalid = 2 * p.I;
+    as1 = as0;
+    as1.base += (long long)XM * as0.ld;
+    as1.rows -= XM;
+    CplxStager<false> bs;
+    bs.base = p.b + ((long long)l * p.ws + n0 / 2) * 2;
+    bs.ldk = p.O;
+    bs.kk_hi = p.I;
+    bs.ovalid = p.O - n0 / 2;
+    const EPI epi0(p, rowbase * 2 * p.O + n0, 2LL * p.O, n0), epi1(p, (rowbase + XM) * 2 * p.O + n0, 2LL * p.O, n0);
+    x3_tile_tall(as0, as1, bs, 0, (2 * p.I + XK - 1) / XK, R - r0, 2 * p.O - n0, epi0, epi1, lds_x3);
+}
+
+template <class EPI>
+__global__ __launch_bounds__(XT, 2) void dhconv_dgrad_x3_tall_kernel(TallPanelParams p) {
+    extern __shared__ __attribute__((aligned(16))) char lds_x3[];
+    const TileId t = decode_block(p.nheavy, p.tiles_m, p.tiles_n);
+    if (!t.valid) return;
+    const int l = p.Lloc - 1 - t.batch;
+    const int R = tri_rows(p.Mloc, p.B, p.l_off, p.m_off, l);
+    const int r0 = t.tm * 2 * XM;
+    if (r0 >= R) return;
+    const int n0 = t.tn * XN;
+    const long long rowbase = (long long)l * p.Mloc * p.B + r0;
+    RowStager as0, as1;
+    as0.base = p.a + rowbase * 2 * p.O;
+    as0.ld = 2 * p.O;
+    as0.rows = R - r0;
+    as0.kvalid = 2 * p.O;
+    as1 = as0;
+    as1.base += (long long)XM * as0.ld;
+    as1.rows -= XM;
+    DgradStager bs;
+    bs.base = p.b + ((long long)l * p.ws + (long long)(n0 / 2) * p.O) * 2;
+    bs.O = p.O;
+    bs.ivalid = p.I - n0 / 2;
+    const EPI epi0(p, rowbase * 2 * p.I + n0, 2LL * p.I, n0), epi1(p, (rowbase + XM) * 2 * p.I + n0, 2LL * p.I, n0);
+    x3_tile_tall(as0, as1, bs, 0, (2 * p.O + XK - 1) / XK, R - r0, 2 * p.I - n0, epi0, epi1, lds_x3);
+}
+
+}
+
+int mk::dhconv_x3_tall_launch(const char* who, bool fwd, const float* a, const float* w, float* dst, int lloc, int mloc, int batch,
+                              int cin, int cout, int l_off, int m_off, int nheavy, void* stream) {
+    TallPanelParams p{panel_params(a, w, dst, lloc, mloc, batch, cin, cout, l_off, m_off, mloc * batch, fwd ? cout : cin), nheavy};
+    p.tiles_m = mk::ceil_div(mloc * batch, 2 * XM);
+    const long long nblk = grid_blocks(nheavy, p.tiles_m, p.tiles_n);
+    return fwd ? x3_launch_tall<dhconv_fwd_x3_tall_kernel<PanelStoreEpi>>(who, nblk, stream, p)
+               : x3_launch_tall<dhconv_dgrad_x3_tall_kernel<PanelStoreEpi>>(who, nblk, stream, p);
+}
```
